# waleedbinkhalid74/cnn-gp

Measured on AMD Instinct MI355X. Metric: kernel entries/s (N×M pairs) + full-Kxx build+solve wall-clock, MNIST 28×28, higher is better.
Workload: dtype f64; 1 GPU; mnist_paper_convnet_gp Kxx 4096x4096, tiles 1024; n=4096, tile=1024, parallelism=tiles-dp1

## Files before the change

cnn-gp_amd/cnn_gp/_native.py:

```python
from __future__ import annotations

import ctypes
import os
import threading

_HERE = os.path.dirname(os.path.abspath(__file__))
LIB_PATH = os.environ.get("CNNGP_LIB",
                          os.path.join(os.path.dirname(_HERE), "lib", "libcnngp.so"))

CGP_ABI_VERSION = 12
CGP_FLAG_EXACT_RELU = 1
CGP_FLAG_GENERIC_CONV = 2
CGP_FLAG_NET_DUAL = 4
CGP_PRE_NONE, CGP_PRE_RELU, CGP_PRE_MOMENTS = 0, 1, 2
CGP_POST_NONE, CGP_POST_RELU = 0, 1
CGP_NET_CONV, CGP_NET_RELU, CGP_NET_MOMENTS, CGP_NET_LINEAR = 0, 1, 2, 3
CGP_NET_LOAD, CGP_NET_STORE = 4, 5
CGP_NET_CODE_HS_CLEAN = 0x100
CGP_NET_CODE_SUM = 0x200
CGP_NET_CODE_FROM_SUM = 0x400
CGP_NET_CODE_GEOMETRY = 0xff
CGP_VAR_MOMENTS, CGP_VAR_CONV, CGP_VAR_HALF, CGP_VAR_SUM = 0, 1, 2, 3
CGP_VAR_FORM_SCALED, CGP_VAR_FORM_RSQRT = 0, 1

_vp = ctypes.c_void_p
_i64 = ctypes.c_int64
_i32 = ctypes.c_int32
_f64 = ctypes.c_double


class ConvArgs(ctypes.Structure):
    _fields_ = [
        ("in_", _vp), ("in_y", _vp), ("out", _vp), ("addend", _vp),
        ("pre_xx", _vp), ("pre_yy", _vp), ("post_xx", _vp), ("post_yy", _vp),
        ("nmaps", _i64), ("n1", _i64), ("n2", _i64),
        ("h", _i32), ("w", _i32), ("ho", _i32), ("wo", _i32),
        ("taps", _i32), ("offset", _i32), ("stride", _i32), ("dilation", _i32),
        ("channels", _i32), ("pre", _i32), ("post", _i32), ("same", _i32), ("diag", _i32),
        ("maps_per_block", _i32), ("flags", _i32), ("reserved", _i32),
        ("weight", _f64), ("bias", _f64),
    ]


class ReluArgs(ctypes.Structure):
    _fields_ = [
        ("xy", _vp), ("out", _vp), ("addend", _vp), ("xx", _vp), ("yy", _vp),
        ("nmaps", _i64), ("n1", _i64), ("n2", _i64),
        ("hw", _i32), ("same", _i32), ("diag", _i32), ("flags", _i32),
    ]


class ReluNtkArgs(ctypes.Structure):
    _fields_ = [
        ("xy", _vp), ("theta", _vp), ("out_xy", _vp), ("out_theta", _vp),
        ("xx", _vp), ("yy", _vp),
        ("nmaps", _i64), ("n1", _i64), ("n2", _i64),
        ("hw", _i32), ("same", _i32), ("diag", _i32), ("flags", _i32),
    ]


class ErfArgs(ctypes.Structure):
    _fields_ = [
        ("xy", _vp), ("theta", _vp), ("out_xy", _vp), ("out_theta", _vp), ("addend", _vp),
        ("xx", _vp), ("yy", _vp),
        ("nmaps", _i64), ("n1", _i64), ("n2", _i64),
        ("hw", _i32), ("same", _i32), ("diag", _i32), ("flags", _i32),
    ]


class NetOp(ctypes.Structure):
    _fields_ = [
        ("kind", _i32), ("code", _i32), ("src", _i32), ("dst", _i32), ("add", _i32),
        ("ws_in", _i32), ("ws_out", _i32), ("relu", _i32), ("h", _i32), ("w", _i32),
        ("div_m", ctypes.c_uint32), ("div_s", ctypes.c_uint32),
        ("dst2", _i32), ("zero_halo", _i32),
        ("weight", _f64), ("bias", _f64), ("var_x", _vp), ("var_y", _vp),
        ("var2_x", _vp), ("var2_y", _vp),
    ]


class VarOp(ctypes.Structure):
    _fields_ = [
        ("kind", _i32), ("dst", _i32), ("src", _i32 * 4),
        ("h", _i32), ("w", _i32), ("ho", _i32), ("wo", _i32),
        ("taps", _i32), ("offset", _i32), ("stride", _i32), ("dilation", _i32),
        ("store", _i64), ("qstore", _i64),
        ("weight", _f64), ("bias", _f64), ("coef", _f64 * 4),
    ]


class VarArgs(ctypes.Structure):
    _fields_ = [
        ("x", _vp), ("y", _vp), ("out", _vp), ("ops", _vp),
        ("n1", _i64), ("n2", _i64), ("store_total", _i64),
        ("nops", _i32), ("channels", _i32), ("h", _i32), ("w", _i32),
        ("lds_elems", _i32), ("scratch", _i32),
    ]


class NetArgs(ctypes.Structure):
    _fields_ = [
        ("x", _vp), ("y", _vp), ("out", _vp), ("kdiag", _vp), ("ops", _vp),
        ("n1", _i64), ("n2", _i64), ("ldo", _i64),
        ("nops", _i32), ("channels", _i32), ("h", _i32), ("w", _i32),
        ("same", _i32), ("final_slot", _i32), ("hs", _i32), ("lds_elems", _i32),
        ("flags", _i32), ("pairs", _i32), ("unit_begin", _i64), ("unit_end", _i64),
        ("final_stage", _i32), ("program", _i32), ("part", _i32),
    ]


def make_fastdiv(d: int):
    s = 0
    while (1 << s) < d:
        s += 1
    m = (((1 << 32) * ((1 << s) - d)) // d + 1) & 0xFFFFFFFF
    return m, s


SIGNATURES = {
    "cgp_abi_version": (_i32, []),
    "cgp_net_xvar_scale": (ctypes.c_double, []),
    "cgp_net_var_form": (_i32, []),
    "cgp_last_error": (ctypes.c_char_p, []),
    "cgp_conv_args_size": (ctypes.c_size_t, []),
    "cgp_relu_args_size": (ctypes.c_size_t, []),
    "cgp_device_count": (_i32, []),
    "cgp_selftest": (_i32, []),
    "cgp_moments_xy_f64": (_i32, [_vp, _vp, _i64, _i64, _i32, _i32, _i32, _vp, _vp]),
    "cgp_moments_xy_f32": (_i32, [_vp, _vp, _i64, _i64, _i32, _i32, _i32, _vp, _vp]),
    "cgp_moments_var_f64": (_i32, [_vp, _vp, _i64, _i64, _i32, _i32, _vp, _vp, _vp]),
    "cgp_moments_var_f32": (_i32, [_vp, _vp, _i64, _i64, _i32, _i32, _vp, _vp, _vp]),
    "cgp_conv_f64": (_i32, [ctypes.POINTER(ConvArgs), _vp]),
    "cgp_conv_f32": (_i32, [ctypes.POINTER(ConvArgs), _vp]),
    "cgp_relu_f64": (_i32, [ctypes.POINTER(ReluArgs), _vp]),
    "cgp_relu_f32": (_i32, [ctypes.POINTER(ReluArgs), _vp]),
    "cgp_relu_ntk_args_size": (ctypes.c_size_t, []),
    "cgp_relu_ntk_f64": (_i32, [ctypes.POINTER(ReluNtkArgs), _vp]),
    "cgp_relu_ntk_f32": (_i32, [ctypes.POINTER(ReluNtkArgs), _vp]),
    "cgp_erf_args_size": (ctypes.c_size_t, []),
    "cgp_erf_f64": (_i32, [ctypes.POINTER(ErfArgs), _vp]),
    "cgp_erf_f32": (_i32, [ctypes.POINTER(ErfArgs), _vp]),
    "cgp_var_erf_f64": (_i32, [_vp, _vp, _i64, _i64, _i32, _i32, _vp, _vp, _vp]),
    "cgp_var_erf_f32": (_i32, [_vp, _vp, _i64, _i64, _i32, _i32, _vp, _vp, _vp]),
    "cgp_var_relu_f64": (_i32, [_vp, _vp, _i64, _i64, _i32, _i32, _vp, _vp, _vp]),
    "cgp_var_relu_f32": (_i32, [_vp, _vp, _i64, _i64, _i32, _i32, _vp, _vp, _vp]),
    "cgp_axpby_f64": (_i32, [_f64, _vp, _f64, _vp, _vp, _i64, _vp]),
    "cgp_axpby_f32": (_i32, [_f64, _vp, _f64, _vp, _vp, _i64, _vp]),
    "cgp_scale_batch_f64": (_i32, [_i32, _vp, _vp, _vp, _f64, _vp]),
    "cgp_rsqrt_batch_f64": (_i32, [_i32, _vp, _vp, _vp, _vp]),
    "cgp_cast_f32_f64": (_i32, [_vp, _vp, _i64, _vp]),
    "cgp_transpose_f64": (_i32, [_vp, _i64, _i64, _vp, _vp]),
    "cgp_chol_solve_f64": (_i32, [_vp, _i64, _i64, _vp, _i64, _i64, _f64,
                                  ctypes.POINTER(_i64), _vp]),
    "cgp_chol_last_phases": (_i32, [_vp, ctypes.POINTER(_f64)]),
    "cgp_chol_solve_f64_timed": (_i32, [_vp, _i64, _i64, _vp, _i64, _i64, _f64,
                                        ctypes.POINTER(_i64), ctypes.POINTER(_f64), _vp]),
    "cgp_gemm_f64": (_i32, [_vp, _vp, _vp, _i64, _i64, _i64, _vp]),
    "cgp_sym_mirror_f64": (_i32, [_vp, _i64, _i64, _vp, _vp]),
    "cgp_sym_residual_f64": (_i32, [_vp, _i64, _i64, _vp, _vp, _vp, _i64, _i64, _vp, _vp]),
    "cgp_argmax_rows_f64": (_i32, [_vp, _i64, _i64, _vp, _vp]),
    "cgp_pred_var_f64": (_i32, [_vp, _i64, _i64, _vp, _i64, _i64, _vp, _vp, _vp]),
    "cgp_net_geometry": (_i32, [_i32] * 7),
    "cgp_net_hs_elems": (_i32, [_i32]),
    "cgp_net_supertile": (_i32, []),
    "cgp_net_units": (_i32, [_i32]),
    "cgp_net_resolution": (_i32, [_i32, _i32]),
    "cgp_net_op_size": (ctypes.c_size_t, []),
    "cgp_net_args_size": (ctypes.c_size_t, []),
    "cgp_net_occupancy": (_i32, [_i32, _i32, _i32, _i32]),
    "cgp_net_program": (_i32, [_vp, _i32, _i32, _i32, _i32, _i32]),
    "cgp_net_validate": (_i32, [_vp, _i32, _i32]),
    "cgp_net_static_lds": (_i32, []),
    "cgp_net_f64": (_i32, [ctypes.POINTER(NetArgs), _vp]),
    "cgp_net_f32": (_i32, [ctypes.POINTER(NetArgs), _vp]),
    "cgp_var_op_size": (ctypes.c_size_t, []),
    "cgp_var_args_size": (ctypes.c_size_t, []),
    "cgp_var_chain_f64": (_i32, [ctypes.POINTER(VarArgs), _vp]),
    "cgp_var_chain_f32": (_i32, [ctypes.POINTER(VarArgs), _vp]),
}

_lib = None
_lib_err = None
_lock = threading.Lock()


def load():
    global _lib, _lib_err
    with _lock:
        if _lib is not None:
            return _lib
        if _lib_err is not None:
            raise RuntimeError(_lib_err)
        if not os.path.exists(LIB_PATH):
            _lib_err = (f"libcnngp.so not found at {LIB_PATH}: build it with "
                        "`python -c 'import __graft_entry__ as g; g.build()'` or "
                        "`make -C cnn-gp_amd/csrc` (no CPU fallback exists)")
            raise RuntimeError(_lib_err)
        try:
            lib = ctypes.CDLL(LIB_PATH)
        except OSError as e:
            _lib_err = f"failed to load {LIB_PATH}: {e}"
            raise RuntimeError(_lib_err) from e
        for name, (res, args) in SIGNATURES.items():
            fn = getattr(lib, name)
            fn.restype = res
            fn.argtypes = args
        if lib.cgp_abi_version() != CGP_ABI_VERSION:
            _lib_err = "libcnngp.so ABI version mismatch (rebuild it)"
            raise RuntimeError(_lib_err)
        if lib.cgp_conv_args_size() != ctypes.sizeof(ConvArgs) or \
                lib.cgp_relu_args_size() != ctypes.sizeof(ReluArgs) or \
                lib.cgp_relu_ntk_args_size() != ctypes.sizeof(ReluNtkArgs) or \
                lib.cgp_erf_args_size() != ctypes.sizeof(ErfArgs) or \
                lib.cgp_net_op_size() != ctypes.sizeof(NetOp) or \
                lib.cgp_net_args_size() != ctypes.sizeof(NetArgs) or \
                lib.cgp_var_op_size() != ctypes.sizeof(VarOp) or \
                lib.cgp_var_args_size() != ctypes.sizeof(VarArgs):
            _lib_err = "libcnngp.so argument struct layout differs from _native.py"
            raise RuntimeError(_lib_err)
        _lib = lib
        return lib


def check(rc: int, what: str):
    if rc != 0:
        msg = load().cgp_last_error().decode(errors="replace")
        raise RuntimeError(f"{what} failed (code {rc}): {msg}")


def call(name: str, *args):
    lib = load()
    check(getattr(lib, name)(*args), name)


def ptr(t):
    return None if t is None else ctypes.c_void_p(t.data_ptr())
```

cnn-gp_amd/csrc/cgp_common.h:

```cpp
#pragma once

#include <hip/hip_runtime.h>

#include <string>

#include "cnngp.h"
#include "relu_poly.h"

namespace cgp {

int fail(int code, const char* fmt, ...);
int check_launch(const char* what);
int device_cus();
inline hipStream_t as_stream(void* s) { return reinterpret_cast<hipStream_t>(s); }
inline hipError_t stream_device(hipStream_t s, int* dev) {
    if (s == nullptr) return hipGetDevice(dev);
    hipDevice_t d = 0;
    const hipError_t e = hipStreamGetDevice(s, &d);
    if (e == hipSuccess) *dev = (int)d;
    return e;
}

#define CGP_HIP(call)                                                                  \
    do {                                                                               \
        hipError_t e_ = (call);                                                        \
        if (e_ != hipSuccess)                                                          \
            return fail(CGP_EHIP, "%s: %s (%s:%d)", #call, hipGetErrorString(e_),      \
                        __FILE__, __LINE__);                                           \
    } while (0)


struct FastDiv {
    unsigned m, s, d;
};
__host__ __device__ inline FastDiv make_fastdiv(unsigned d) {
    FastDiv f;
    f.d = d;
    f.s = 0;
    while ((1ull << f.s) < d) ++f.s;
    f.m = (unsigned)(((1ull << 32) * ((1ull << f.s) - d)) / d + 1);
    return f;
}
__host__ __device__ __forceinline__ unsigned umulhi32(unsigned a, unsigned b) {
#ifdef __HIP_DEVICE_COMPILE__
    return __umulhi(a, b);
#else
    return (unsigned)(((unsigned long long)a * b) >> 32);
#endif
}
__host__ __device__ __forceinline__ unsigned fdiv(unsigned n, const FastDiv& f) {
    return (umulhi32(n, f.m) + n) >> f.s;
}

template <typename T> struct K;
template <> struct K<double> {
    static constexpr double pi = 3.141592653589793;
    static constexpr double two_pi = 6.283185307179586;
    static constexpr double tiny = 1.1754943508222875e-38;
    static constexpr double xfloor = 1e-300;
};
template <> struct K<float> {
    static constexpr float pi = 3.14159265358979f;
    static constexpr float two_pi = 6.28318530717959f;
    static constexpr float tiny = 1.17549435e-38f;
    static constexpr float xfloor = 1e-30f;
};

__device__ __forceinline__ double sqrt_t(double x) { return __builtin_sqrt(x); }
__device__ __forceinline__ float sqrt_t(float x) { return __builtin_sqrtf(x); }
__device__ __forceinline__ double acos_t(double x) { return acos(x); }
__device__ __forceinline__ float acos_t(float x) { return acosf(x); }

template <typename T>
__device__ __forceinline__ T relu_exact_inl(T c, T v1, T v2) {
    const T t = v1 * v2 + K<T>::tiny;
    T cs = c * (T(1) / sqrt_t(t));
    cs = cs < T(-1) ? T(-1) : (cs > T(1) ? T(1) : cs);
    T d = t - c * c;
    d = d < T(0) ? T(0) : d;
    const T s = sqrt_t(d);
    const T th = acos_t(cs);
    return (s + (K<T>::pi - th) * c) / K<T>::two_pi;
}
template <typename T>
__device__ __noinline__ T relu_exact(T c, T v1, T v2) {
    return relu_exact_inl(c, v1, v2);
}

__device__ __forceinline__ double rsqrt_fast(double t) {
    const double y = __builtin_amdgcn_rsq(t);
    const double e = __builtin_fma(-t * y, y, 1.0);
    return __builtin_fma(0.5 * y, e, y);
}
__device__ __forceinline__ float rsqrt_fast(float t) { return __builtin_amdgcn_rsqf(t); }
__device__ __forceinline__ double sqrt_fast(double x) {
    const double r = __builtin_amdgcn_rsq(x);
    const double s0 = x * r;
    return __builtin_fma(0.5 * r, __builtin_fma(-s0, s0, x), s0);
}
__device__ __forceinline__ float sqrt_fast(float x) { return x * __builtin_amdgcn_rsqf(x); }
__device__ __forceinline__ double relu_poly(double x) {
    double r = kReluPolyD[kReluPolyDegD];
#pragma unroll
    for (int k = kReluPolyDegD - 1; k >= 0; --k) r = __builtin_fma(r, x, kReluPolyD[k]);
    return r;
}
__device__ __forceinline__ float relu_poly(float x) {
    float r = kReluPolyF[kReluPolyDegF];
#pragma unroll
    for (int k = kReluPolyDegF - 1; k >= 0; --k) r = __builtin_fmaf(r, x, kReluPolyF[k]);
    return r;
}
__device__ __forceinline__ double fmin_t(double a, double b) { return __builtin_fmin(a, b); }
__device__ __forceinline__ float fmin_t(float a, float b) { return __builtin_fminf(a, b); }
__device__ __forceinline__ double fmax_t(double a, double b) { return __builtin_fmax(a, b); }
__device__ __forceinline__ float fmax_t(float a, float b) { return __builtin_fmaxf(a, b); }
__device__ __forceinline__ double fabs_t(double a) { return __builtin_fabs(a); }
__device__ __forceinline__ float fabs_t(float a) { return __builtin_fabsf(a); }
__device__ __forceinline__ double fma_t(double a, double b, double c) {
    return __builtin_fma(a, b, c);
}
__device__ __forceinline__ float fma_t(float a, float b, float c) {
    return __builtin_fmaf(a, b, c);
}

constexpr double kXVarScale = 0.0625;
#ifndef CGP_RELU_ONE_ROOT
#define CGP_RELU_ONE_ROOT 1
#endif
constexpr int kNetVarForm = CGP_RELU_ONE_ROOT ? CGP_VAR_FORM_RSQRT : CGP_VAR_FORM_SCALED;
constexpr double kPolyQ = CGP_RELU_ONE_ROOT ? 0.5 : 0.125;
__device__ __forceinline__ double var_rsqrt8(double v) { return 1.0 / __builtin_sqrt(v * 0.125); }
constexpr double kYMax = 0x1p66;
constexpr double poly_q(int k) {
    double v = kReluPolyD[k] * kPolyQ;
    for (int n = 0; n < k; ++n) v *= 0.25;
    return v;
}
struct PolyCoef {
    double c[kReluPolyDegD + 1];
};
constexpr PolyCoef poly_coef(bool quartered) {
    PolyCoef t{};
    for (int k = 0; k <= kReluPolyDegD; ++k) t.c[k] = quartered ? poly_q(k) : kReluPolyD[k];
    return t;
}
static __constant__ PolyCoef kReluPolyTabD = poly_coef(false);
static __constant__ PolyCoef kReluPolyTabDq = poly_coef(true);

template <int D>
struct AdaptCoef {
    double c[D + 1];
};
template <int D>
constexpr AdaptCoef<D> adapt_coef(const double (&p)[D + 1]) {
    AdaptCoef<D> t{};
    for (int k = 0; k <= D; ++k) {
        double v = p[k] * kPolyQ;
        for (int n = 0; n < k; ++n) v *= 0.25;
        t.c[k] = v;
    }
    return t;
}
static __constant__ AdaptCoef<kReluAdaptDeg0> kReluAdaptTab0 = adapt_coef<kReluAdaptDeg0>(kReluAdaptP0);
static __constant__ AdaptCoef<kReluAdaptDeg1> kReluAdaptTab1 = adapt_coef<kReluAdaptDeg1>(kReluAdaptP1);
static __constant__ AdaptCoef<kReluAdaptDeg2> kReluAdaptTab2 = adapt_coef<kReluAdaptDeg2>(kReluAdaptP2);

typedef const __attribute__((address_space(4))) double* ConstD;
struct PolyTab {
    ConstD d, dq;
    ConstD a0, a1, a2;
};
__device__ __forceinline__ PolyTab poly_table() {
    ConstD p = (ConstD)kReluPolyTabD.c;
    ConstD q = (ConstD)kReluPolyTabDq.c;
    asm volatile("" : "+s"(p), "+s"(q));
    ConstD a0 = (ConstD)kReluAdaptTab0.c;
    ConstD a1 = (ConstD)kReluAdaptTab1.c;
    ConstD a2 = (ConstD)kReluAdaptTab2.c;
    asm volatile("" : "+s"(a0), "+s"(a1), "+s"(a2));
    return PolyTab{p, q, a0, a1, a2};
}
__device__ __forceinline__ double fma_sc(double r, double u, double c) {
    double o;
    asm("v_fma_f64 %0, %1, %2, %3" : "=v"(o) : "v"(r), "v"(u), "s"(c));
    return o;
}
__device__ __forceinline__ double relu_poly(double x, const PolyTab& t) {
    double r = fma_sc(t.d[kReluPolyDegD], x, t.d[kReluPolyDegD - 1]);
#pragma unroll
    for (int k = kReluPolyDegD - 2; k >= 0; --k) r = fma_sc(r, x, t.d[k]);
    return r;
}
__device__ __forceinline__ float relu_poly(float x, const PolyTab&) { return relu_poly(x); }

template <typename T>
__device__ __forceinline__ T relu_fast(T c, T v1, T v2, const PolyTab& tab) {
    const T t = fma_t(v1, v2, K<T>::tiny);
    const T y = rsqrt_fast(t);
    const T st = t * y;
    const T a = fmin_t(fabs_t(c * y), T(1));
    const T x = fma_t(T(-0.5), a, T(0.5));
    const T sx = sqrt_fast(fmax_t(x, K<T>::xfloor));
    const T p = relu_poly(x, tab);
    const T hpos = (c + fabs_t(c)) * T(0.25);
    return fma_t((st * x) * sx, p, hpos);
}

constexpr double kRhoMax = 1.0 - 0x1p-52;
template <int R>
__device__ __forceinline__ void relu_fast_n(double (&c)[R], const double (&v1)[R],
                                            const double (&v2)[R], const PolyTab& tab) {
    double y[R], st[R], a[R], sx[R], u[R], p[R];
#pragma unroll
    for (int r = 0; r < R; ++r) {
        const double t = __builtin_fma(v1[r], v2[r], K<double>::tiny);
        y[r] = rsqrt_fast(t);
        st[r] = t * y[r];
    }
#pragma unroll
    for (int r = 0; r < R; ++r) {
        a[r] = __builtin_fmin(__builtin_fabs(c[r] * y[r]), kRhoMax);
        u[r] = __builtin_fma(-0.5, a[r], 0.5);
        sx[r] = (st[r] * u[r]) * sqrt_fast(u[r]);
    }
#pragma unroll
    for (int r = 0; r < R; ++r) p[r] = fma_sc(tab.d[kReluPolyDegD], u[r], tab.d[kReluPolyDegD - 1]);
#pragma unroll
    for (int k = kReluPolyDegD - 2; k >= 0; --k) {
        const double ck = tab.d[k];
#pragma unroll
        for (int r = 0; r < R; ++r) p[r] = fma_sc(p[r], u[r], ck);
    }
#pragma unroll
    for (int r = 0; r < R; ++r)
        c[r] = __builtin_fma(sx[r], p[r], (c[r] + __builtin_fabs(c[r])) * 0.25);
}
template <int R, int D>
__device__ __forceinline__ void horner_q(double (&p)[R], const double (&u)[R], ConstD t) {
#pragma unroll
    for (int r = 0; r < R; ++r) p[r] = fma_sc(t[D], u[r], t[D - 1]);
#pragma unroll
    for (int k = D - 2; k >= 0; --k) {
        const double ck = t[k];
#pragma unroll
        for (int r = 0; r < R; ++r) p[r] = fma_sc(p[r], u[r], ck);
    }
}
#ifndef CGP_RELU_VOTE_HI
#define CGP_RELU_VOTE_HI 1
#endif
__device__ __forceinline__ unsigned vote_hi(double v) {
    return (unsigned)(__builtin_bit_cast(unsigned long long, v) >> 32);
}
template <int R>
__device__ __forceinline__ unsigned vote_hi_max(const double (&u)[R]) {
    unsigned m = vote_hi(u[0]);
#pragma unroll
    for (int r = 1; r < R; ++r) m = m > vote_hi(u[r]) ? m : vote_hi(u[r]);
    return m;
}
template <int R, bool QIN, int AD = 0>
__device__ __forceinline__ void relu_q_n(double (&c)[R], const double (&v1q)[R],
                                         const double (&v2)[R], const PolyTab& tab,
                                         unsigned long long seg = ~0ull) {
    double sx[R], u[R], p[R];
#if CGP_RELU_ONE_ROOT
    double Y[R];
#pragma unroll
    for (int r = 0; r < R; ++r) {
        if constexpr (!QIN) c[r] *= 0.25;
        Y[r] = __builtin_fmin(v1q[r] * v2[r], kYMax);
    }
#pragma unroll
    for (int r = 0; r < R; ++r) {
        u[r] = __builtin_fmax(__builtin_fma(-__builtin_fabs(c[r]), Y[r], 2.0), 2.0 - 2.0 * kRhoMax);
        const double z = (u[r] * Y[r]) * Y[r];
        const double h = __builtin_amdgcn_rsq(z);
        const double m = z * h;
        const double R2 = h * __builtin_fma(-m, h, 3.0);
        sx[r] = (u[r] * u[r]) * R2;
    }
#else
    double y[R], st[R];
#pragma unroll
    for (int r = 0; r < R; ++r) {
        if constexpr (!QIN) c[r] *= 0.25;
        const double T = __builtin_fma(v1q[r], v2[r], kXVarScale * K<double>::tiny);
        const double r0 = __builtin_amdgcn_rsq(T);
        const double m = T * r0;
        const double k = __builtin_fma(-m, r0, 3.0);
        y[r] = r0 * k;
        st[r] = m * k;
    }
#pragma unroll
    for (int r = 0; r < R; ++r) {
        u[r] = __builtin_fmax(__builtin_fma(-__builtin_fabs(c[r]), y[r], 2.0), 2.0 - 2.0 * kRhoMax);
        const double h = __builtin_amdgcn_rsq(u[r]);
        const double m = u[r] * h;
        const double sq4 = m * __builtin_fma(-m, h, 3.0);
        sx[r] = (st[r] * u[r]) * sq4;
    }
#endif
    if constexpr (AD == 2) {
        const unsigned long long ex = __builtin_amdgcn_read_exec() & seg;
        auto all_seg = [&](bool pred) { return (__ballot(pred) & seg) == ex; };
#if CGP_RELU_VOTE_HI
        const unsigned hm = vote_hi_max<R>(u);
        if (all_seg(hm < vote_hi(4.0 * kReluAdaptX0))) {
            horner_q<R, kReluAdaptDeg0>(p, u, tab.a0);
        } else if (all_seg(hm < vote_hi(4.0 * kReluAdaptX1))) {
            horner_q<R, kReluAdaptDeg1>(p, u, tab.a1);
        } else if (all_seg(hm < vote_hi(4.0 * kReluAdaptX2))) {
#else
        double um = u[0];
#pragma unroll
        for (int r = 1; r < R; ++r) um = __builtin_fmax(um, u[r]);
        if (all_seg(um <= 4.0 * kReluAdaptX0)) {
            horner_q<R, kReluAdaptDeg0>(p, u, tab.a0);
        } else if (all_seg(um <= 4.0 * kReluAdaptX1)) {
            horner_q<R, kReluAdaptDeg1>(p, u, tab.a1);
        } else if (all_seg(um <= 4.0 * kReluAdaptX2)) {
#endif
            horner_q<R, kReluAdaptDeg2>(p, u, tab.a2);
        } else {
            horner_q<R, kReluPolyDegD>(p, u, tab.dq);
        }
    } else if constexpr (AD == 1) {
#if CGP_RELU_VOTE_HI
        const unsigned hm = vote_hi_max<R>(u);
        if (__all(hm < vote_hi(4.0 * kReluAdaptX0))) {
            horner_q<R, kReluAdaptDeg0>(p, u, tab.a0);
        } else if (__all(hm < vote_hi(4.0 * kReluAdaptX1))) {
            horner_q<R, kReluAdaptDeg1>(p, u, tab.a1);
        } else if (__all(hm < vote_hi(4.0 * kReluAdaptX2))) {
#else
        double um = u[0];
#pragma unroll
        for (int r = 1; r < R; ++r) um = __builtin_fmax(um, u[r]);
        if (__all(um <= 4.0 * kReluAdaptX0)) {
            horner_q<R, kReluAdaptDeg0>(p, u, tab.a0);
        } else if (__all(um <= 4.0 * kReluAdaptX1)) {
            horner_q<R, kReluAdaptDeg1>(p, u, tab.a1);
        } else if (__all(um <= 4.0 * kReluAdaptX2)) {
#endif
            horner_q<R, kReluAdaptDeg2>(p, u, tab.a2);
        } else {
            horner_q<R, kReluPolyDegD>(p, u, tab.dq);
        }
    } else {
        horner_q<R, kReluPolyDegD>(p, u, tab.dq);
    }
#pragma unroll
    for (int r = 0; r < R; ++r) c[r] = __builtin_fma(sx[r], p[r], c[r] + __builtin_fabs(c[r]));
}
typedef float cgp_f2 __attribute__((ext_vector_type(2)));
__device__ __forceinline__ cgp_f2 relu_fast2(cgp_f2 c, cgp_f2 v1, cgp_f2 v2) {
    const cgp_f2 t = __builtin_elementwise_fma(v1, v2, cgp_f2(K<float>::tiny));
    const cgp_f2 y = {__builtin_amdgcn_rsqf(t.x), __builtin_amdgcn_rsqf(t.y)};
    const cgp_f2 st = t * y;
    const cgp_f2 cy = c * y;
    const cgp_f2 a = {__builtin_fminf(__builtin_fabsf(cy.x), 1.0f),
                      __builtin_fminf(__builtin_fabsf(cy.y), 1.0f)};
    const cgp_f2 x = __builtin_elementwise_fma(cgp_f2(-0.5f), a, cgp_f2(0.5f));
    const cgp_f2 xm = {__builtin_fmaxf(x.x, K<float>::xfloor), __builtin_fmaxf(x.y, K<float>::xfloor)};
    const cgp_f2 h = {__builtin_amdgcn_rsqf(xm.x), __builtin_amdgcn_rsqf(xm.y)};
    const cgp_f2 sx = xm * h;
    cgp_f2 p = cgp_f2(kReluPolyF[kReluPolyDegF]);
#pragma unroll
    for (int k = kReluPolyDegF - 1; k >= 0; --k)
        p = __builtin_elementwise_fma(p, x, cgp_f2(kReluPolyF[k]));
    const cgp_f2 ac = {__builtin_fabsf(c.x), __builtin_fabsf(c.y)};
    const cgp_f2 hpos = (c + ac) * cgp_f2(0.25f);
    return __builtin_elementwise_fma((st * x) * sx, p, hpos);
}
__device__ __forceinline__ void relu_prep2(cgp_f2 c, cgp_f2 v1, cgp_f2 v2, cgp_f2& x, cgp_f2& m,
                                           cgp_f2& hpos) {
    const cgp_f2 t = __builtin_elementwise_fma(v1, v2, cgp_f2(K<float>::tiny));
    const cgp_f2 y = {__builtin_amdgcn_rsqf(t.x), __builtin_amdgcn_rsqf(t.y)};
    const cgp_f2 st = t * y;
    const cgp_f2 cy = c * y;
    const cgp_f2 a = {__builtin_fminf(__builtin_fabsf(cy.x), 1.0f),
                      __builtin_fminf(__builtin_fabsf(cy.y), 1.0f)};
    x = __builtin_elementwise_fma(cgp_f2(-0.5f), a, cgp_f2(0.5f));
    const cgp_f2 xm = {__builtin_fmaxf(x.x, K<float>::xfloor), __builtin_fmaxf(x.y, K<float>::xfloor)};
    const cgp_f2 h = {__builtin_amdgcn_rsqf(xm.x), __builtin_amdgcn_rsqf(xm.y)};
    m = (st * x) * (xm * h);
    const cgp_f2 ac = {__builtin_fabsf(c.x), __builtin_fabsf(c.y)};
    hpos = (c + ac) * cgp_f2(0.25f);
}
__device__ __forceinline__ void relu_prep1(float c, float v1, float v2, float& x, float& m,
                                           float& hpos) {
    const float t = __builtin_fmaf(v1, v2, K<float>::tiny);
    const float y = __builtin_amdgcn_rsqf(t);
    const float st = t * y;
    const float a = __builtin_fminf(__builtin_fabsf(c * y), 1.0f);
    x = __builtin_fmaf(-0.5f, a, 0.5f);
    const float xm = __builtin_fmaxf(x, K<float>::xfloor);
    m = (st * x) * (xm * __builtin_amdgcn_rsqf(xm));
    hpos = (c + __builtin_fabsf(c)) * 0.25f;
}
template <int R, int D>
__device__ __forceinline__ void relu_poly_f(const float (&P)[D + 1], float (&c)[R],
                                            const cgp_f2 (&x2)[R / 2 + 1],
                                            const cgp_f2 (&m2)[R / 2 + 1],
                                            const cgp_f2 (&h2)[R / 2 + 1], float xs, float ms,
                                            float hs) {
#pragma unroll
    for (int q = 0; q < R / 2; ++q) {
        cgp_f2 p = cgp_f2(P[D]);
#pragma unroll
        for (int k = D - 1; k >= 0; --k) p = __builtin_elementwise_fma(p, x2[q], cgp_f2(P[k]));
        const cgp_f2 o = __builtin_elementwise_fma(m2[q], p, h2[q]);
        c[2 * q] = o.x;
        c[2 * q + 1] = o.y;
    }
    if constexpr (R % 2) {
        float p = P[D];
#pragma unroll
        for (int k = D - 1; k >= 0; --k) p = __builtin_fmaf(p, xs, P[k]);
        c[R - 1] = __builtin_fmaf(ms, p, hs);
    }
}
template <int R>
__device__ __forceinline__ void relu_fast_n(float (&c)[R], const float (&v1)[R],
                                            const float (&v2)[R], const PolyTab&) {
    cgp_f2 x2[R / 2 + 1], m2[R / 2 + 1], h2[R / 2 + 1];
    float xs = 0.0f, ms = 0.0f, hs = 0.0f;
#pragma unroll
    for (int q = 0; q < R / 2; ++q)
        relu_prep2(cgp_f2{c[2 * q], c[2 * q + 1]}, cgp_f2{v1[2 * q], v1[2 * q + 1]},
                   cgp_f2{v2[2 * q], v2[2 * q + 1]}, x2[q], m2[q], h2[q]);
    if constexpr (R % 2) relu_prep1(c[R - 1], v1[R - 1], v2[R - 1], xs, ms, hs);
    relu_poly_f<R, kReluPolyDegF>(kReluPolyF, c, x2, m2, h2, xs, ms, hs);
}

template <typename T>
__device__ __forceinline__ T relu_fast(T c, T v1, T v2) {
    const T t = v1 * v2 + K<T>::tiny;
    const T y = rsqrt_fast(t);
    const T st = t * y;
    const T a = fmin_t(fabs_t(c * y), T(1));
    const T x = fma_t(T(-0.5), a, T(0.5));
    const T sx = sqrt_fast(fmax_t(x, K<T>::xfloor));
    const T p = relu_poly(x);
    const T pos = fmax_t(c, T(0));
    return fma_t((st * x) * sx, p, T(0.5) * pos) + (c - c);
}

template <typename T>
__device__ __forceinline__ T relu_pair(T c, const T* __restrict__ xx, const T* __restrict__ yy,
                                       unsigned i, unsigned j, int hw, int px, int same,
                                       int diag, int exact) {
    const T v1 = xx[(size_t)i * hw + px];
    if (same && (diag || i == j)) return v1 / T(2);
    const T v2 = yy[(size_t)j * hw + px];
    return exact ? relu_exact(c, v1, v2) : relu_fast(c, v1, v2);
}

__device__ __forceinline__ double atan_t(double x) { return atan(x); }
__device__ __forceinline__ float atan_t(float x) { return atanf(x); }

template <typename T> struct KErf {
    static constexpr T two_over_pi = T(0.63661977236758134308);
    static constexpr T four_over_pi = T(1.27323954473516268615);
};

template <typename T>
__device__ __forceinline__ T erf_var(T v, T& kdot) {
    const T s = sqrt_t(T(1) + T(4) * v);
    kdot = KErf<T>::four_over_pi / s;
    return KErf<T>::two_over_pi * atan_t((T(2) * v) / s);
}
template <typename T>
__device__ __forceinline__ T erf_var(T v) {
    T kdot;
    return erf_var(v, kdot);
}

template <typename T>
__device__ __forceinline__ T erf_pair(T c, const T* __restrict__ xx, const T* __restrict__ yy,
                                      unsigned i, unsigned j, int hw, int px, int same,
                                      int diag, T& kdot) {
    const T v1 = xx[(size_t)i * hw + px];
    if (same && (diag || i == j)) return erf_var(v1, kdot);
    const T v2 = yy[(size_t)j * hw + px];
    T d = T(1) + T(2) * (v1 + v2) + T(4) * (v1 * v2 - c * c);
    d = d < T(1) ? T(1) : d;
    const T s = sqrt_t(d);
    kdot = KErf<T>::four_over_pi / s;
    return KErf<T>::two_over_pi * atan_t((T(2) * c) / s);
}

__device__ __forceinline__ void pair_of(unsigned m, const FastDiv& n2, int diag, unsigned& i,
                                        unsigned& j) {
    if (diag) {
        i = j = m;
    } else {
        i = fdiv(m, n2);
        j = m - i * n2.d;
    }
}

__device__ __forceinline__ void lds_barrier() {
    asm volatile("s_waitcnt lgkmcnt(0)" ::: "memory");
    __builtin_amdgcn_s_barrier();
    asm volatile("" ::: "memory");
}

}
```

cnn-gp_amd/csrc/netfuse.hip:

```cpp

#include "cgp_common.h"


#include <map>
#include <mutex>
#include <utility>
#include <algorithm>
#include <climits>

using namespace cgp;

namespace {

constexpr int kNT = 128;
constexpr int kSplit = 2;
template <int NP>
constexpr int kNTof = NP == 2 ? kSplit * kNT : kNT;
template <int NP>
constexpr int kUnitsOf = NP == 2 ? kSplit : NP;
constexpr int kSTL = 3;
constexpr int kST = 1 << kSTL;
constexpr int kEw = 4;

constexpr int pick_r(int lines, int len, int taps, int s, int epi, int nt) {
    int best = 1;
    long long best_cost = LLONG_MAX;
    for (int r = 1; r <= 8 && r <= len; ++r) {
        if (len % r) continue;
        const int items = lines * (len / r);
        const int rounds = (items + nt - 1) / nt;
        const long long cost = (long long)rounds * (epi * r + (r - 1) * s + taps);
        if (cost < best_cost || (cost == best_cost && r > best)) {
            best = r;
            best_cost = cost;
        }
    }
    return best;
}

template <int H_, int W_, int HO_, int WO_, int TAPS_, int S_, int OFF_, int NP_ = 1>
struct NG {
    static constexpr int H = H_, W = W_, HO = HO_, WO = WO_, TAPS = TAPS_, S = S_, OFF = OFF_;
    static constexpr int NP = NP_;
    static constexpr int NT = kNT;
    static_assert(NP_ != 2, "two-pair workgroups run their ops as one-pair halves");
    static constexpr int HW = H * W, HOWO = HO * WO;
    static constexpr bool POINT = TAPS == 1 && OFF == 0;
    static constexpr bool REDUCE = HO == 1 && WO == 1 && OFF == 0 && TAPS == H && TAPS == W;
    static constexpr int HSR = (HO - 1) * S + TAPS;
    static constexpr int Q0 = OFF < 0 ? -OFF : 0;
    static constexpr int Q1 = HSR < H - OFF ? HSR : H - OFF;
    static constexpr int NVR = Q1 - Q0;
    static constexpr int R2 = pick_r(NVR * NP, WO, TAPS, S, 2, NT);
    static constexpr int R3 = pick_r(WO * NP, HO, TAPS, S, 8, NT);
    static constexpr int WIN2 = (R2 - 1) * S + TAPS, WIN3 = (R3 - 1) * S + TAPS;
    static constexpr int NG2 = WO / R2, NH = NVR * NG2, KH = (NP * NH + NT - 1) / NT;
    static constexpr int NG3 = HO / R3, NV = NG3 * WO, KV = (NP * NV + NT - 1) / NT;
    static constexpr int NZ = (HSR - NVR) * WO;
    static constexpr bool DIRECT = !POINT && !REDUCE && TAPS <= 3;
    static constexpr int HS_ELEMS = (POINT || REDUCE || DIRECT) ? 2 : HSR * WO;
};

#define CGP_NET_GEOMETRIES(X)          \
    X(28, 28, 28, 28, 7, 1, -3)        \
    X(28, 28, 28, 28, 4, 1, -1)        \
    X(28, 28, 28, 28, 3, 1, -1)        \
    X(28, 28, 28, 28, 1, 1, 0)         \
    X(28, 28, 14, 14, 3, 2, -1)        \
    X(28, 28, 14, 14, 1, 2, 0)         \
    X(28, 28, 1, 1, 28, 1, 0)          \
    X(14, 14, 14, 14, 3, 1, -1)        \
    X(14, 14, 7, 7, 3, 2, -1)          \
    X(14, 14, 7, 7, 1, 2, 0)           \
    X(7, 7, 7, 7, 3, 1, -1)            \
    X(7, 7, 1, 1, 7, 1, 0)             \
    X(1, 1, 1, 1, 1, 1, 0)             \
    X(32, 32, 32, 32, 3, 1, -1)        \
    X(32, 32, 32, 32, 1, 1, 0)         \
    X(32, 32, 16, 16, 3, 2, -1)        \
    X(32, 32, 16, 16, 1, 2, 0)         \
    X(16, 16, 16, 16, 3, 1, -1)        \
    X(16, 16, 8, 8, 3, 2, -1)          \
    X(16, 16, 8, 8, 1, 2, 0)           \
    X(8, 8, 8, 8, 3, 1, -1)            \
    X(8, 8, 1, 1, 8, 1, 0)             \
    X(14, 14, 1, 1, 14, 1, 0)          \
    X(16, 16, 1, 1, 16, 1, 0)          \
    X(32, 32, 1, 1, 32, 1, 0)

struct GeoRow {
    int h, w, ho, wo, taps, s, off, hs_elems;
};
#define CGP_NET_ROW(h, w, ho, wo, k, s, o) {h, w, ho, wo, k, s, o, NG<h, w, ho, wo, k, s, o>::HS_ELEMS},
constexpr GeoRow kGeoTable[] = {CGP_NET_GEOMETRIES(CGP_NET_ROW)};
#undef CGP_NET_ROW
constexpr int kNumGeo = sizeof(kGeoTable) / sizeof(kGeoTable[0]);

template <typename T, int TAPS, int O0, int G, int N, int R>
__device__ __forceinline__ void win_group(const T (&w)[N], T (&out)[R]) {
    T core = w[O0 + G - 1];
#pragma unroll
    for (int t = O0 + G; t < O0 + TAPS; ++t) core += w[t];
    if constexpr (G == 1) {
        out[O0] = core;
    } else {
        T suf[G], right[G];
        suf[G - 1] = core;
#pragma unroll
        for (int o = G - 2; o >= 0; --o) suf[o] = w[O0 + o] + suf[o + 1];
        right[1] = w[O0 + TAPS];
#pragma unroll
        for (int o = 2; o < G; ++o) right[o] = right[o - 1] + w[O0 + TAPS + o - 1];
        out[O0] = suf[0];
#pragma unroll
        for (int o = 1; o < G; ++o) out[O0 + o] = suf[o] + right[o];
    }
}

template <typename T, int TAPS, int O0, int N, int R>
__device__ __forceinline__ void win_groups(const T (&w)[N], T (&out)[R]) {
    if constexpr (O0 < R) {
        constexpr int G = (R - O0) < TAPS ? (R - O0) : TAPS;
        win_group<T, TAPS, O0, G, N, R>(w, out);
        win_groups<T, TAPS, O0 + TAPS, N, R>(w, out);
    }
}

template <typename T, int TAPS, int S, int R>
__device__ __forceinline__ void win_sums(const T (&w)[(R - 1) * S + TAPS], T (&out)[R]) {
    if constexpr (S == 1 && TAPS >= 4 && R > 1) {
        win_groups<T, TAPS, 0, (R - 1) * S + TAPS, R>(w, out);
    } else {
#pragma unroll
        for (int o = 0; o < R; ++o) {
            T acc = w[o * S];
#pragma unroll
            for (int t = 1; t < TAPS; ++t) acc += w[o * S + t];
            out[o] = acc;
        }
    }
}

__device__ __forceinline__ int opaque_tid() {
    static_assert(kNT == 128, "opaque_tid masks to 128-thread halves");
    int t;
    asm volatile("v_and_b32 %0, 0x7f, %1" : "=v"(t) : "v"((int)threadIdx.x));
    return t;
}

__device__ __forceinline__ int udiv(int a, int d) { return (int)((unsigned)a / (unsigned)d); }

typedef const cgp_net_op* OpsC;
__device__ __forceinline__ OpsC ops_c(const cgp_net_op* p) { return (OpsC)p; }
__device__ __forceinline__ cgp_net_op load_op(OpsC r) {
    cgp_net_op o;
    o.kind = r->kind;
    o.code = r->code;
    o.src = r->src;
    o.dst = r->dst;
    o.add = r->add;
    o.ws_in = r->ws_in;
    o.ws_out = r->ws_out;
    o.relu = r->relu;
    o.h = r->h;
    o.w = r->w;
    o.div_m = r->div_m;
    o.div_s = r->div_s;
    o.dst2 = r->dst2;
    o.zero_halo = r->zero_halo;
    o.weight = r->weight;
    o.bias = r->bias;
    o.var_x = r->var_x;
    o.var_y = r->var_y;
    o.var2_x = r->var2_x;
    o.var2_y = r->var2_y;
    return o;
}

template <typename T>
using GP = const __attribute__((address_space(1))) T*;
template <typename T>
__device__ __forceinline__ GP<T> gptr(const void* p) {
    return (GP<T>)(const T*)p;
}

template <typename T>
__device__ __forceinline__ T wave_sum(T v) {
#pragma unroll
    for (int m = 32; m >= 1; m >>= 1) v += __shfl_xor(v, m, 64);
    return v;
}

template <typename T>
struct NetP {
    const T* __restrict__ x;
    const T* __restrict__ y;
    T* __restrict__ out;
    const T* __restrict__ kdiag;
    const cgp_net_op* __restrict__ ops;
    unsigned long long* work;
    long long ldo, units, ubeg, uend;
    unsigned n1, n2, nbi, nbj;
    int nops, channels, hw_in, same, final_slot, hs, lds_elems, exact, final_stage, part;
};

constexpr int kMaxNP = 16;
constexpr long long kStaticLds = 1536;
struct Pairs {
    unsigned i, j;
    const unsigned* tab;
    long long u0;
    void* red;
};
template <int NP>
__device__ __forceinline__ void pair_q(const Pairs& pr, int q, unsigned& iq, unsigned& jq) {
    if constexpr (NP == 1) {
        iq = pr.i;
        jq = pr.j;
    } else {
        iq = pr.tab[q];
        jq = pr.tab[kMaxNP + q];
    }
}

template <bool EXACT, typename T>
__device__ __forceinline__ T relu_of(T c, T v1, T v2, const PolyTab& tab) {
    if constexpr (EXACT)
        return relu_exact_inl(c, v1, v2);
    else
        return relu_fast(c, v1, v2, tab);
}
template <typename T, bool EX>
constexpr bool kQuarter = !EX && sizeof(T) == 8;

template <bool EXACT, bool QIN, typename T, int R, int AD = 0>
__device__ __forceinline__ void relu_n(T (&v)[R], const T (&u1)[R], const T (&u2)[R],
                                       const PolyTab& tab, unsigned long long seg = ~0ull) {
    if constexpr (EXACT) {
#pragma unroll
        for (int k = 0; k < R; ++k) v[k] = relu_exact_inl(v[k], u1[k], u2[k]);
    } else if constexpr (sizeof(T) == 8) {
        relu_q_n<R, QIN, AD>(v, u1, u2, tab, seg);
    } else {
        relu_fast_n<R>(v, u1, u2, tab);
    }
}

#define CGP_NET_RESOLUTIONS(X) X(28, 28) X(14, 14) X(7, 7) X(32, 32) X(16, 16) X(8, 8) X(1, 1)

struct ResRow {
    int h, w;
};
#define CGP_NET_RES_ROW(h, w) {h, w},
constexpr ResRow kResTable[] = {CGP_NET_RESOLUTIONS(CGP_NET_RES_ROW)};
#undef CGP_NET_RES_ROW
constexpr int kNumRes = sizeof(kResTable) / sizeof(kResTable[0]);
constexpr int res_index(int h, int w) {
    for (int n = 0; n < kNumRes; ++n)
        if (kResTable[n].h == h && kResTable[n].w == w) return n;
    return -1;
}

template <typename T, bool EX, bool DU, int R, int AD = 0>
__device__ __forceinline__ void net_out(T* __restrict__ lds, const cgp_net_op& op, T (&v)[R],
                                        const int (&at)[R], const bool (&ok)[R],
                                        const T (&u1)[R], const T (&u2)[R],
                                        const PolyTab& tab, unsigned long long seg = ~0ull) {
    if (op.relu) relu_n<EX, kQuarter<T, EX>, T, R, AD>(v, u1, u2, tab, seg);
    if (op.add >= 0) {
#pragma unroll
        for (int k = 0; k < R; ++k)
            if (ok[k]) v[k] += lds[op.add + at[k]];
    }
#pragma unroll
    for (int k = 0; k < R; ++k)
        if (ok[k]) lds[op.dst + at[k]] = v[k];
    if (DU && op.dst2 >= 0) {
        relu_n<EX, false, T, R, AD>(v, u1, u2, tab, seg);
#pragma unroll
        for (int k = 0; k < R; ++k)
            if (ok[k]) lds[op.dst2 + at[k]] = v[k];
    }
}

__device__ __forceinline__ GP<char> ubase(const void* p) {
    const unsigned long long v = (unsigned long long)p;
    const unsigned lo = __builtin_amdgcn_readfirstlane((unsigned)v);
    const unsigned hi = __builtin_amdgcn_readfirstlane((unsigned)(v >> 32));
    return (GP<char>)(const char*)(((unsigned long long)hi << 32) | lo);
}

template <typename T>
struct VarSrc {
    GP<char> x, y;
    unsigned xo, yo;
    bool on;
    __device__ __forceinline__ T ldx(unsigned px, int k = 0) const {
        return *(GP<T>)(x + (size_t)(xo + px * (unsigned)sizeof(T)) + k * (int)sizeof(T));
    }
    __device__ __forceinline__ T ldy(unsigned px, int k = 0) const {
        return *(GP<T>)(y + (size_t)(yo + px * (unsigned)sizeof(T)) + k * (int)sizeof(T));
    }
};
template <typename T, bool UNI>
__device__ __forceinline__ VarSrc<T> var_maps(const void* vx, const void* vy, bool on,
                                              unsigned i, unsigned j, int hw) {
    VarSrc<T> r;
    r.on = on;
    r.x = ubase(vx);
    r.y = ubase(vy);
    if constexpr (UNI) {
        r.x += (size_t)i * (size_t)hw * sizeof(T);
        r.y += (size_t)j * (size_t)hw * sizeof(T);
        r.xo = r.yo = 0;
    } else {
        r.xo = i * (unsigned)hw * (unsigned)sizeof(T);
        r.yo = j * (unsigned)hw * (unsigned)sizeof(T);
    }
    return r;
}
template <typename T, bool UNI>
__device__ __forceinline__ VarSrc<T> var_src(const cgp_net_op& op, unsigned i, unsigned j,
                                             int hw) {
    const bool two = op.dst2 >= 0;
    return var_maps<T, UNI>(two ? op.var2_x : op.var_x, two ? op.var2_y : op.var_y,
                            op.relu != 0 || two, i, j, hw);
}

template <int NP>
constexpr int kAdaptOf = NP == 1 ? 1 : 2;
constexpr int kPrio = 2;
constexpr int kPrioMaxHW = 28 * 28;
template <int NP, int HW>
constexpr bool kPrioOn = HW <= kPrioMaxHW;
template <int NP, int HW>
__device__ __forceinline__ void prio_mem() {
    if constexpr (kPrioOn<NP, HW>) __builtin_amdgcn_s_setprio(kPrio);
}
template <int NP, int HW>
__device__ __forceinline__ void prio_alu() {
    if constexpr (kPrioOn<NP, HW>) __builtin_amdgcn_s_setprio(0);
}
template <int PER, int NPR>
struct VoteCuts {
    int n = 0;
    int at[64] = {};
    constexpr VoteCuts() {
        for (int off = 1; off < PER && n < 64; ++off) {
            bool cut = false;
            for (int k = 1; 64 * k < NPR * PER; ++k) cut = cut || (64 * k) % PER == off;
            if (cut) at[n++] = off;
        }
    }
};
template <int PER, int NPR>
__device__ __forceinline__ unsigned long long vote_lanes(int it) {
    constexpr VoteCuts<PER, NPR> cuts{};
    const int wb = it & ~63, q = udiv(it, PER), l = it - q * PER;
    int lo = 0, hi = PER;
#pragma unroll
    for (int k = 0; k < cuts.n; ++k) {
        if (cuts.at[k] <= l) lo = cuts.at[k];
        if (cuts.at[k] > l && cuts.at[k] < hi) hi = cuts.at[k];
    }
    int a = q * PER + lo - wb, b = q * PER + hi - wb;
    a = a < 0 ? 0 : a;
    b = b > 64 ? 64 : b;
    const unsigned long long top = b >= 64 ? ~0ull : ((1ull << b) - 1ull);
    return top & ~((1ull << a) - 1ull);
}
#ifndef CGP_NET_RES_UNDEF
#define CGP_NET_RES_UNDEF 1
#endif
template <typename T, bool EX, bool DU, class G, bool PRE = false>
__device__ __forceinline__ void net_conv(T* __restrict__ lds, const cgp_net_op& op,
                                         const NetP<T>& p, const Pairs& pr) {
    constexpr int NP = G::NP;
    const int tid = opaque_tid();
    const PolyTab tab = poly_table();
    const T qs = !PRE && kQuarter<T, EX> && op.relu ? T(0.25) : T(1);
    const T w = T(op.weight) * qs, b = T(op.bias) * qs;
    const int arena = NP == 1 ? 0 : p.lds_elems;
    prio_mem<NP, G::HW>();
    const VarSrc<T> vs0 = var_src<T, NP == 1>(op, pr.i, pr.j, G::HOWO);
    auto vs_of = [&](int q) {
        if constexpr (NP == 1) {
            return vs0;
        } else {
            unsigned iq, jq;
            pair_q<NP>(pr, q, iq, jq);
            return var_src<T, false>(op, iq, jq, G::HOWO);
        }
    };
    const T* __restrict__ src = lds + op.src;
    const int wsi = op.ws_in, wso = op.ws_out;

    if constexpr (G::REDUCE && NP == 1) {
        prio_alu<NP, G::HW>();
        const bool from_sum = (op.code & CGP_NET_CODE_FROM_SUM) != 0;
        T* part = from_sum ? static_cast<T*>(pr.red)
                           : lds + p.part;
        if (!from_sum) {
            T acc = T(0);
#pragma unroll
            for (int k = 0; k < (G::HW + G::NT - 1) / G::NT; ++k) {
                const int px = tid + k * G::NT;
                if (G::HW % G::NT == 0 || px < G::HW) {
                    const int r = udiv(px, G::W), c = px - r * G::W;
                    acc += src[r * wsi + c];
                }
            }
            acc = wave_sum(acc);
            if ((tid & 63) == 0) part[tid >> 6] = acc;
            lds_barrier();
        }
        if (tid == 0) {
            T tot = part[0];
#pragma unroll
            for (int k = 1; k < G::NT / 64; ++k) tot += part[k];
            T v[1] = {fma_t(w, tot, b)};
            const int at[1] = {0};
            const bool ok[1] = {true};
            T u1[1] = {T(1)}, u2[1] = {T(1)};
            if (vs0.on) {
                u1[0] = vs0.ldx(0);
                u2[0] = vs0.ldy(0);
            }
            net_out<T, EX, DU, 1>(lds, op, v, at, ok, u1, u2, tab);
        }
    } else if constexpr (G::REDUCE) {
        prio_alu<NP, G::HW>();
        constexpr int TPP = G::NT / NP;
        static_assert(TPP <= 64 && G::NT % NP == 0, "reduce groups must not straddle waves");
        const int q = udiv(tid, TPP), lane = tid - q * TPP;
        const T* srcq = src + q * arena;
        T acc = T(0);
#pragma unroll
        for (int k = 0; k < (G::HW + TPP - 1) / TPP; ++k) {
            const int px = lane + k * TPP;
            if (G::HW % TPP == 0 || px < G::HW) {
                const int r = udiv(px, G::W), c = px - r * G::W;
                acc += srcq[r * wsi + c];
            }
        }
#pragma unroll
        for (int m = TPP / 2; m >= 1; m >>= 1) acc += __shfl_xor(acc, m, 64);
        if (lane == 0) {
            const VarSrc<T> vs = vs_of(q);
            T v[1] = {fma_t(w, acc, b)};
            const int at[1] = {q * arena};
            const bool ok[1] = {true};
            T u1[1] = {T(1)}, u2[1] = {T(1)};
            if (vs.on) {
                u1[0] = vs.ldx(0);
                u2[0] = vs.ldy(0);
            }
            net_out<T, EX, DU, 1>(lds, op, v, at, ok, u1, u2, tab);
        }
    } else if constexpr (G::POINT) {
        prio_alu<NP, G::HW>();
        constexpr int N = NP * G::HOWO;
        constexpr int KP = (N + G::NT - 1) / G::NT;
        T u1[KP], u2[KP], v[KP];
        int at[KP];
        bool ok[KP];
#pragma unroll
        for (int k = 0; k < KP; ++k) {
            const int e = tid + k * G::NT;
            ok[k] = N % G::NT == 0 || e < N;
            const int ec = ok[k] ? e : 0;
            const int q = NP == 1 ? 0 : udiv(ec, G::HOWO), pc = ec - q * G::HOWO;
            const int r = udiv(pc, G::WO), c = pc - r * G::WO;
            const VarSrc<T> vs = vs_of(q);
            at[k] = q * arena + r * wso + c;
            u1[k] = (vs.on && ok[k]) ? vs.ldx((unsigned)pc) : T(1);
            u2[k] = (vs.on && ok[k]) ? vs.ldy((unsigned)pc) : T(1);
            v[k] = fma_t(w, src[q * arena + (r * G::S) * wsi + c * G::S], b);
        }
        net_out<T, EX, DU, KP, NP == 1 ? 1 : 0>(lds, op, v, at, ok, u1, u2, tab);
    } else if constexpr (G::DIRECT) {
        constexpr int NVT = NP * G::NV;
        T u1[G::KV][G::R3], u2[G::KV][G::R3];
#pragma unroll
        for (int kv = 0; kv < G::KV; ++kv) {
            const int it = tid + kv * G::NT;
            const int itc = (NVT % G::NT == 0 || it < NVT) ? it : 0;
            const int q = NP == 1 ? 0 : udiv(itc, G::NV), l = itc - q * G::NV;
            const int g3 = udiv(l, G::WO), c = l - g3 * G::WO;
            const VarSrc<T> vs = vs_of(q);
#pragma unroll
            for (int k = 0; k < G::R3; ++k) {
                const unsigned px0 = (unsigned)(g3 * G::R3 * G::WO + c);
                u1[kv][k] = vs.on ? vs.ldx(px0, k * G::WO) : T(1);
                u2[kv][k] = vs.on ? vs.ldy(px0, k * G::WO) : T(1);
            }
        }
        const int s_lo = op.src - wsi, s_hi = op.src + G::H * wsi;
        auto hits = [&](int d) {
            return d >= 0 && d - wso < s_hi && d + G::HO * wso > s_lo;
        };
        const bool hazard = hits(op.dst) || (DU && hits(op.dst2));
        T res[G::KV][G::R3];
#if CGP_NET_RES_UNDEF
#pragma unroll
        for (int kv = 0; kv < G::KV; ++kv)
#pragma unroll
            for (int k = 0; k < G::R3; ++k) asm volatile("" : "=v"(res[kv][k]));
#endif
#pragma unroll
        for (int kv = 0; kv < G::KV; ++kv) {
            const int it = tid + kv * G::NT;
            if (NVT % G::NT == 0 || it < NVT) {
                const int q = NP == 1 ? 0 : udiv(it, G::NV), l = it - q * G::NV;
                const int g3 = udiv(l, G::WO), c = l - g3 * G::WO;
                const T* base = src + q * arena + c * G::S + G::OFF;
                const int r0 = g3 * G::R3 * G::S + G::OFF;
                T rs[G::WIN3];
#pragma unroll
                for (int t = 0; t < G::WIN3; ++t) {
                    const bool lo = G::OFF + t < 0, hi = (G::NG3 - 1) * G::R3 * G::S + G::OFF + t >= G::H;
                    const int r = r0 + t;
                    const bool in = (!lo || r >= 0) && (!hi || r < G::H);
                    const T* row = base + (in ? r : 0) * wsi;
                    T a = row[0];
#pragma unroll
                    for (int dx = 1; dx < G::TAPS; ++dx) a += row[dx];
                    rs[t] = in ? a : T(0);
                }
                T o[G::R3];
                win_sums<T, G::TAPS, G::S, G::R3>(rs, o);
#pragma unroll
                for (int k = 0; k < G::R3; ++k) res[kv][k] = fma_t(w, o[k], b);
#pragma unroll
                for (int k = 0; k < G::R3; ++k)
                    asm volatile("" : "+v"(u1[kv][k]), "+v"(u2[kv][k]));
            }
        }
        prio_alu<NP, G::HW>();
        if (hazard) lds_barrier();
#pragma unroll
        for (int kv = 0; kv < G::KV; ++kv) {
            const int it = tid + kv * G::NT;
            if (NVT % G::NT == 0 || it < NVT) {
                const int q = NP == 1 ? 0 : udiv(it, G::NV), l = it - q * G::NV;
                const int g3 = udiv(l, G::WO), c = l - g3 * G::WO;
                int at[G::R3];
                bool ok[G::R3];
#pragma unroll
                for (int k = 0; k < G::R3; ++k) {
                    at[k] = q * arena + (g3 * G::R3 + k) * wso + c;
                    ok[k] = true;
                }
                net_out<T, EX, DU, G::R3, kAdaptOf<NP>>(lds, op, res[kv], at, ok, u1[kv],
                                                        u2[kv], tab,
                                                        NP == 1 ? ~0ull : vote_lanes<G::NV, NP>(it));
            }
        }
    } else {
        T* __restrict__ hs = lds + p.hs;
        constexpr int NHT = NP * G::NH, NVT = NP * G::NV, NZT = NP * G::NZ;
        T u1[G::KV][G::R3], u2[G::KV][G::R3];
        if (vs0.on) {
#pragma unroll
            for (int kv = 0; kv < G::KV; ++kv) {
                const int it = tid + kv * G::NT;
                const int itc = (NVT % G::NT == 0 || it < NVT) ? it : 0;
                const int q = NP == 1 ? 0 : udiv(itc, G::NV), l = itc - q * G::NV;
                const int g3 = udiv(l, G::WO), c = l - g3 * G::WO;
                const VarSrc<T> vs = vs_of(q);
#pragma unroll
                for (int k = 0; k < G::R3; ++k) {
                    const unsigned px0 = (unsigned)(g3 * G::R3 * G::WO + c);
                    u1[kv][k] = vs.ldx(px0, k * G::WO);
                    u2[kv][k] = vs.ldy(px0, k * G::WO);
                }
            }
        } else {
#pragma unroll
            for (int kv = 0; kv < G::KV; ++kv)
#pragma unroll
                for (int k = 0; k < G::R3; ++k) u1[kv][k] = u2[kv][k] = T(1);
        }
#pragma unroll
        for (int kh = 0; kh < G::KH; ++kh) {
            const int it = tid + kh * G::NT;
            if (NHT % G::NT == 0 || it < NHT) {
                const int q = NP == 1 ? 0 : udiv(it, G::NH), l = it - q * G::NH;
                const int qi = udiv(l, G::NG2), g2 = l - qi * G::NG2;
                const T* row = lds + (op.src + q * arena + (G::Q0 + qi + G::OFF) * wsi +
                                      g2 * G::R2 * G::S + G::OFF);
                T win[G::WIN2];
#pragma unroll
                for (int t = 0; t < G::WIN2; ++t) win[t] = row[t];
                T o[G::R2];
                win_sums<T, G::TAPS, G::S, G::R2>(win, o);
                T* h = hs + q * arena + (G::Q0 + qi) * G::WO + g2 * G::R2;
#pragma unroll
                for (int t = 0; t < G::R2; ++t) h[t] = o[t];
            }
        }
        if constexpr (G::NZ > 0) {
            if (!(op.code & CGP_NET_CODE_HS_CLEAN)) {
#pragma unroll
                for (int z0 = 0; z0 < NZT; z0 += G::NT) {
                    const int z = z0 + tid;
                    if (NZT % G::NT == 0 || z < NZT) {
                        const int q = NP == 1 ? 0 : udiv(z, G::NZ), zl = z - q * G::NZ;
                        hs[q * arena + (zl < G::Q0 * G::WO ? zl : zl + G::NVR * G::WO)] = T(0);
                    }
                }
            }
        }
        lds_barrier();
        const bool to_sum = NP == 1 && (op.code & CGP_NET_CODE_SUM) != 0;
        T sacc = T(0);
#pragma unroll
        for (int kv = 0; kv < G::KV; ++kv) {
            const int it = tid + kv * G::NT;
            if (NVT % G::NT == 0 || it < NVT) {
                const int q = NP == 1 ? 0 : udiv(it, G::NV), l = it - q * G::NV;
                const int g3 = udiv(l, G::WO), c = l - g3 * G::WO;
                const T* col = lds + (p.hs + q * arena + g3 * G::R3 * G::S * G::WO + c);
                T win[G::WIN3];
#pragma unroll
                for (int t = 0; t < G::WIN3; ++t) win[t] = col[t * G::WO];
#pragma unroll
                for (int k = 0; k < G::R3; ++k) asm volatile("" : "+v"(u1[kv][k]), "+v"(u2[kv][k]));
                T o[G::R3], v[G::R3];
                win_sums<T, G::TAPS, G::S, G::R3>(win, o);
                prio_alu<NP, G::HW>();
                int at[G::R3];
                bool ok[G::R3];
#pragma unroll
                for (int k = 0; k < G::R3; ++k) {
                    v[k] = fma_t(w, o[k], b);
                    at[k] = q * arena + (g3 * G::R3 + k) * wso + c;
                    ok[k] = true;
                }
                if (to_sum) {
                    if (op.relu) relu_n<EX, kQuarter<T, EX>, T, G::R3, 1>(v, u1[kv], u2[kv], tab);
#pragma unroll
                    for (int k = 0; k < G::R3; ++k) sacc += v[k];
                } else {
                    net_out<T, EX, DU, G::R3, kAdaptOf<NP>>(lds, op, v, at, ok, u1[kv], u2[kv],
                                                            tab,
                                                            NP == 1 ? ~0ull
                                                                    : vote_lanes<G::NV, NP>(it));
                }
            }
        }
        if constexpr (NP == 1) {
            if (to_sum) {
                sacc = wave_sum(sacc);
                if ((tid & 63) == 0) static_cast<T*>(pr.red)[tid >> 6] = sacc;
            }
        }
    }
}

template <typename T, bool EX, bool DU, int KIND, int KE, int W_, int NP>
__device__ __forceinline__ void elem_pass(T* __restrict__ lds, const cgp_net_op& op,
                                          const NetP<T>& p, const Pairs& pr, int tid,
                                          int base, int hw, const PolyTab& tab) {
    static_assert(NP == 1 || W_ > 0, "multi-pair elementwise ops need a compile-time size");
    const int wd = W_ ? W_ : op.w, ws = op.ws_out;
    const int arena = NP == 1 ? 0 : p.lds_elems;
    const FastDiv fw{op.div_m, op.div_s, (unsigned)op.w};
    auto vs_of = [&](unsigned iq, unsigned jq) {
        return KIND == CGP_NET_RELU
                   ? var_maps<T, NP == 1>(op.var_x, op.var_y, true, iq, jq, hw)
                   : var_src<T, NP == 1>(op, iq, jq, hw);
    };
    const VarSrc<T> vs0 = vs_of(pr.i, pr.j);
    const GP<char> xi = ubase(p.x) + (size_t)pr.i * p.channels * hw * sizeof(T);
    const GP<char> yj = ubase(p.y) + (size_t)pr.j * p.channels * hw * sizeof(T);
    auto img = [](GP<char> b, unsigned e) {
        return *(GP<T>)(b + (size_t)(e * (unsigned)sizeof(T)));
    };
    const int n = NP * hw;
    const bool live = base + (tid & ~63) < n;
    T a[KE], u1[KE], u2[KE];
    int at[KE];
    bool ok[KE];
#pragma unroll
    for (int k = 0; k < KE; ++k) {
        const int e = base + k * kNT + tid;
        ok[k] = e < n;
        const int ec = ok[k] ? e : 0;
        const int q = NP == 1 ? 0 : ec / hw, pc = ec - q * hw;
        const int r = W_ ? udiv(pc, W_) : (int)fdiv((unsigned)pc, fw);
        at[k] = q * arena + r * ws + (pc - r * wd);
        VarSrc<T> vs = vs0;
        if constexpr (NP > 1) {
            unsigned iq, jq;
            pair_q<NP>(pr, q, iq, jq);
            vs = vs_of(iq, jq);
        }
        u1[k] = (vs.on && ok[k]) ? vs.ldx((unsigned)pc) : T(1);
        u2[k] = (vs.on && ok[k]) ? vs.ldy((unsigned)pc) : T(1);
        if constexpr (KIND == CGP_NET_RELU) {
            a[k] = lds[op.src + at[k]];
        } else if constexpr (KIND == CGP_NET_MOMENTS) {
            static_assert(NP == 1, "moments run one pair per workgroup (half)");
            T acc = img(xi, (unsigned)pc) * img(yj, (unsigned)pc);
            for (int ch = 1; ch < p.channels; ++ch) {
                const unsigned e = (unsigned)(ch * hw + pc);
                acc += img(xi, e) * img(yj, e);
            }
            a[k] = acc;
        } else {
            a[k] = T(op.weight) * lds[op.src + at[k]] + T(op.bias) * lds[op.add + at[k]];
        }
    }
    if constexpr (KIND == CGP_NET_MOMENTS) {
        if (p.channels != 1) {
#pragma unroll
            for (int k = 0; k < KE; ++k) a[k] = a[k] / T(p.channels);
        }
    }
    if constexpr (KIND == CGP_NET_RELU) {
        if (live) relu_n<EX, false, T, KE, NP == 1 ? 1 : 0>(a, u1, u2, tab);
        if (op.add >= 0) {
#pragma unroll
            for (int k = 0; k < KE; ++k)
                if (ok[k]) a[k] += lds[op.add + at[k]];
        }
    }
#pragma unroll
    for (int k = 0; k < KE; ++k)
        if (ok[k]) lds[op.dst + at[k]] = a[k];
    if constexpr (KIND == CGP_NET_LINEAR && DU) {
        if (op.dst2 >= 0) {
            if (live) relu_n<EX, false, T, KE, NP == 1 ? 1 : 0>(a, u1, u2, tab);
#pragma unroll
            for (int k = 0; k < KE; ++k)
                if (ok[k]) lds[op.dst2 + at[k]] = a[k];
        }
    }
}

template <typename T, bool EX, bool DU, int KIND, int H_, int W_, int NP, int PI>
__device__ __forceinline__ void elem_passes(T* __restrict__ lds, const cgp_net_op& op,
                                            const NetP<T>& p, const Pairs& pr, int tid,
                                            const PolyTab& tab) {
    constexpr int KF = (NP * H_ * W_ + kNT - 1) / kNT;
    if constexpr (PI * kEw < KF) {
        constexpr int KE = KF - PI * kEw < kEw ? KF - PI * kEw : kEw;
        elem_pass<T, EX, DU, KIND, KE, W_, NP>(lds, op, p, pr, tid, PI * kEw * kNT, H_ * W_,
                                               tab);
        elem_passes<T, EX, DU, KIND, H_, W_, NP, PI + 1>(lds, op, p, pr, tid, tab);
    }
}

template <typename T, bool EX, bool DU, int KIND, int H_, int W_, int NP>
__device__ __forceinline__ void net_elem(T* __restrict__ lds, const cgp_net_op& op,
                                         const NetP<T>& p, const Pairs& pr) {
    const int tid = opaque_tid();
    const PolyTab tab = poly_table();
    if constexpr (H_ == 0) {
        const int hw = op.h * op.w;
        for (int base = 0; base < hw; base += kEw * kNT)
            elem_pass<T, EX, DU, KIND, kEw, 0, 1>(lds, op, p, pr, tid, base, hw, tab);
    } else {
        elem_passes<T, EX, DU, KIND, H_, W_, NP, 0>(lds, op, p, pr, tid, tab);
    }
}

template <typename T, int KIND, int NP>
__device__ __forceinline__ void net_move(T* __restrict__ lds, const cgp_net_op& op,
                                         const NetP<T>& p, const Pairs& pr) {
    const int tid = opaque_tid();
    const int hw = op.h * op.w, n = NP * hw;
    const int arena = NP == 1 ? 0 : p.lds_elems;
    T* state = const_cast<T*>(static_cast<const T*>(op.var_x));
    for (int e = tid; e < n; e += kNT) {
        const int q = NP == 1 ? 0 : e / hw, l = e - q * hw;
        const int r = l / op.w, c = l - r * op.w;
        const size_t g = (size_t)(pr.u0 + q - p.ubeg) * (size_t)op.code + (size_t)op.add +
                         (size_t)l;
        if constexpr (KIND == CGP_NET_LOAD)
            lds[op.dst + q * arena + r * op.ws_out + c] = state[g];
        else
            state[g] = lds[op.src + q * arena + r * op.ws_in + c];
    }
}

#ifndef CGP_NET_MOVE_C
#define CGP_NET_MOVE_C 1
#endif
template <typename T, int KIND, int NP, int H_, int W_, int SLOT, int WS>
__device__ __forceinline__ void net_move_c(T* __restrict__ lds, const cgp_net_op& op,
                                           const NetP<T>& p, const Pairs& pr) {
    const int tid = opaque_tid();
    constexpr int HW = H_ * W_, N = NP * HW, KP = (N + kNT - 1) / kNT;
    const int arena = NP == 1 ? 0 : p.lds_elems;
    const unsigned long long u0 =
        ((unsigned long long)__builtin_amdgcn_readfirstlane((unsigned)((unsigned long long)pr.u0 >> 32)) << 32) |
        __builtin_amdgcn_readfirstlane((unsigned)pr.u0);
    const unsigned code = (unsigned)__builtin_amdgcn_readfirstlane(op.code);
    const GP<char> base = ubase(op.var_x) +
                          ((size_t)(u0 - (unsigned long long)p.ubeg) * code + (size_t)op.add) *
                              sizeof(T);
#pragma unroll
    for (int k = 0; k < KP; ++k) {
        const int e = k * kNT + tid;
        if (N % kNT == 0 || e < N) {
            const unsigned q = NP == 1 ? 0u : (unsigned)udiv(e, HW);
            const unsigned l = (unsigned)e - q * (unsigned)HW;
            const unsigned r = (unsigned)udiv((int)l, W_), c = l - r * (unsigned)W_;
            T* cell = lds + (SLOT + (int)q * arena + (int)(r * (unsigned)WS + c));
            typedef __attribute__((address_space(1))) T* GW;
            GW g = (GW)(base + (size_t)((q * code + l) * (unsigned)sizeof(T)));
            if constexpr (KIND == CGP_NET_LOAD)
                *cell = *g;
            else
                *g = *cell;
        }
    }
}

template <typename T, int NT>
__device__ __forceinline__ void zero_halos(T* lds, int origin, int code, int h, int w, int ws,
                                           int tid) {
    if (!code) return;
    const int hl = code >> 8, gap = code & 0xff;
    for (int e = tid; e < hl + h * gap; e += NT) {
        int cell;
        if (e < hl) {
            cell = origin - hl + e;
        } else {
            const int r = (e - hl) / gap;
            cell = origin + r * ws + w + (e - hl - r * gap);
        }
        lds[cell] = T(0);
    }
}

__device__ __forceinline__ void tri_decode(unsigned s, unsigned nb, unsigned& bi,
                                           unsigned& bj) {
    const double a = 2.0 * nb + 1.0;
    long long r = (long long)((a - sqrt(a * a - 8.0 * (double)s)) * 0.5);
    auto off = [nb](long long q) { return q * (long long)nb - q * (q - 1) / 2; };
    if (r < 0) r = 0;
    while (r > 0 && off(r) > (long long)s) --r;
    while (off(r + 1) <= (long long)s) ++r;
    bi = (unsigned)r;
    bj = (unsigned)(r + ((long long)s - off(r)));
}

template <typename T>
__device__ __forceinline__ bool unit_pair(const NetP<T>& p, long long u, unsigned& i,
                                          unsigned& j) {
    const unsigned s = (unsigned)(u >> (2 * kSTL)), q = (unsigned)u & (kST * kST - 1u);
    unsigned bi, bj;
    if (p.same) {
        tri_decode(s, p.nbi, bi, bj);
    } else {
        bi = s / p.nbj;
        bj = s - bi * p.nbj;
    }
    i = bi * kST + (q >> kSTL);
    j = bj * kST + (q & (kST - 1u));
    return u < p.units && i < p.n1 && j < p.n2;
}

constexpr int geo_index(int h, int w, int ho, int wo, int k, int s, int o) {
    for (int n = 0; n < kNumGeo; ++n) {
        const GeoRow& g = kGeoTable[n];
        if (g.h == h && g.w == w && g.ho == ho && g.wo == wo && g.taps == k && g.s == s &&
            g.off == o)
            return n;
    }
    return -1;
}

#define CGP_NET_FITS(h, w) (NP == 1 || (h) * (w) * NP <= 1024)

#define CGP_NET_CASE(h, w, ho, wo, k, s, o)                                          \
    case geo_index(h, w, ho, wo, k, s, o):                                           \
        if constexpr (CGP_NET_FITS(h, w))                                            \
            net_conv<T, EX, DU, NG<h, w, ho, wo, k, s, o, NP>>(lds, op, p, pr);      \
        break;

#define CGP_NET_RES_CASE(h, w)                                                        \
    case res_index(h, w):                                                             \
        if constexpr (CGP_NET_FITS(h, w)) net_elem<T, EX, DU, KIND, h, w, NP>(lds, op, p, pr); \
        break;

template <typename T, bool EX, bool DU, int KIND, int NP>
__device__ __forceinline__ void net_elem_dispatch(T* __restrict__ lds, const cgp_net_op& op,
                                                  const NetP<T>& p, const Pairs& pr) {
    if constexpr (KIND == CGP_NET_RELU || (KIND == CGP_NET_LINEAR && NP > 1)) {
        switch (op.code) {
            CGP_NET_RESOLUTIONS(CGP_NET_RES_CASE)
        default:
            if constexpr (NP == 1) net_elem<T, EX, DU, KIND, 0, 0, 1>(lds, op, p, pr);
            break;
        }
    } else if constexpr (NP == 1) {
        net_elem<T, EX, DU, KIND, 0, 0, 1>(lds, op, p, pr);
    }
}

template <typename T, bool EX, bool DU, int NP>
__device__ __forceinline__ void net_op(T* __restrict__ lds, const cgp_net_op& op,
                                       const NetP<T>& p, const Pairs& pr, int tid) {
    if (op.zero_halo) {
#pragma unroll
        for (int q = 0; q < NP; ++q) {
            const int qa = NP == 1 ? 0 : q * p.lds_elems;
            zero_halos<T, kNT>(lds + qa, op.dst, op.zero_halo & 0xffff, op.h, op.w,
                                     op.ws_out, tid);
            zero_halos<T, kNT>(lds + qa, op.dst2, (unsigned)op.zero_halo >> 16, op.h, op.w,
                       op.ws_out, tid);
        }
    }
    switch (op.kind) {
    case CGP_NET_CONV:
        switch (op.code & CGP_NET_CODE_GEOMETRY) {
            CGP_NET_GEOMETRIES(CGP_NET_CASE)
        default:
            break;
        }
        break;
    case CGP_NET_RELU:
        net_elem_dispatch<T, EX, DU, CGP_NET_RELU, NP>(lds, op, p, pr);
        break;
    case CGP_NET_MOMENTS:
        net_elem_dispatch<T, EX, DU, CGP_NET_MOMENTS, NP>(lds, op, p, pr);
        break;
    case CGP_NET_LINEAR:
        net_elem_dispatch<T, EX, DU, CGP_NET_LINEAR, NP>(lds, op, p, pr);
        break;
    case CGP_NET_LOAD:
        net_move<T, CGP_NET_LOAD, NP>(lds, op, p, pr);
        break;
    case CGP_NET_STORE:
        net_move<T, CGP_NET_STORE, NP>(lds, op, p, pr);
        break;
    default:
        break;
    }
}

#ifndef CGP_NET_PRESCALE
#define CGP_NET_PRESCALE 1
#endif
constexpr bool kNetPrescale = CGP_NET_PRESCALE != 0;
struct ProgOp {
    int kind, code, src, dst, add, ws_in, ws_out, relu, h, w, dst2, zero_halo;
};
struct ProgInfo {
    int first, nops, pairs, dual, lds_elems, sizes;
};
#include "net_programs.h"
constexpr int kNumProgs = sizeof(kProgs) / sizeof(kProgs[0]);

struct ProgRec {
    double weight, bias;
    const void* var_x;
    const void* var_y;
    const void* var2_x;
    const void* var2_y;
};
template <int PID>
constexpr int kRecsOf = PID >= 0 ? kProgs[PID < 0 ? 0 : PID].nops : 1;

template <int PID, int K>
__device__ __forceinline__ cgp_net_op prog_op(const ProgRec* recs) {
    constexpr ProgOp o = kProgOps[kProgs[PID].first + K];
    const ProgRec& rt = recs[K];
    cgp_net_op op;
    op.kind = o.kind;
    op.code = o.code;
    op.src = o.src;
    op.dst = o.dst;
    op.add = o.add;
    op.ws_in = o.ws_in;
    op.ws_out = o.ws_out;
    op.relu = o.relu;
    op.h = o.h;
    op.w = o.w;
    op.div_m = 0;
    op.div_s = 0;
    op.dst2 = o.dst2;
    op.zero_halo = o.zero_halo;
    op.weight = rt.weight;
    op.bias = rt.bias;
    op.var_x = rt.var_x;
    op.var_y = rt.var_y;
    op.var2_x = rt.var2_x;
    op.var2_y = rt.var2_y;
    return op;
}
template <int PID, int K, int NP>
struct ProgGeo {
    static constexpr ProgOp o = kProgOps[kProgs[PID].first + K];
    static constexpr GeoRow g = kGeoTable[o.code & CGP_NET_CODE_GEOMETRY];
    using G = NG<g.h, g.w, g.ho, g.wo, g.taps, g.s, g.off, NP>;
};
template <typename T, bool DU, int NP, int PID, int K>
__device__ __forceinline__ void prog_ops(T* __restrict__ lds, const NetP<T>& p, const Pairs& pr,
                                         int tid, const ProgRec* recs) {
    constexpr ProgInfo I = kProgs[PID];
    if constexpr (K < I.nops) {
        constexpr ProgOp o = kProgOps[I.first + K];
        const cgp_net_op op = prog_op<PID, K>(recs);
        if constexpr (o.zero_halo != 0) {
#pragma unroll
            for (int q = 0; q < NP; ++q) {
                const int qa = q * I.lds_elems;
                zero_halos<T, kNT>(lds + qa, o.dst, o.zero_halo & 0xffff, o.h, o.w,
                                         o.ws_out, tid);
                zero_halos<T, kNT>(lds + qa, o.dst2, (unsigned)o.zero_halo >> 16, o.h, o.w,
                                         o.ws_out,
                           tid);
            }
        }
        if constexpr (o.kind == CGP_NET_CONV) {
            net_conv<T, false, DU, typename ProgGeo<PID, K, NP>::G, kNetPrescale>(lds, op, p,
                                                                                 pr);
        } else if constexpr (o.kind == CGP_NET_RELU || o.kind == CGP_NET_LINEAR ||
                             o.kind == CGP_NET_MOMENTS) {
            net_elem<T, false, DU, o.kind, o.h, o.w, NP>(lds, op, p, pr);
        } else if constexpr (o.kind == CGP_NET_LOAD || o.kind == CGP_NET_STORE) {
            if constexpr (CGP_NET_MOVE_C)
                net_move_c<T, o.kind, NP, o.h, o.w, o.kind == CGP_NET_LOAD ? o.dst : o.src,
                           o.kind == CGP_NET_LOAD ? o.ws_out : o.ws_in>(lds, op, p, pr);
            else
                net_move<T, o.kind, NP>(lds, op, p, pr);
        }
        lds_barrier();
        prog_ops<T, DU, NP, PID, K + 1>(lds, p, pr, tid, recs);
    }
}

int prog_match(const cgp_net_op* ops, int nops, int pairs, int dual, int lds_elems,
               int itemsize) {
    for (int k = 0; k < kNumProgs; ++k) {
        const ProgInfo& I = kProgs[k];
        if (I.nops != nops || I.pairs != pairs || I.dual != dual || I.lds_elems != lds_elems ||
            !(I.sizes & itemsize))
            continue;
        bool eq = true;
        for (int n = 0; n < nops && eq; ++n) {
            const ProgOp& o = kProgOps[I.first + n];
            const cgp_net_op& r = ops[n];
            eq = o.kind == r.kind && o.code == r.code && o.src == r.src && o.dst == r.dst &&
                 o.add == r.add && o.ws_in == r.ws_in && o.ws_out == r.ws_out &&
                 o.relu == r.relu && o.h == r.h && o.w == r.w && o.dst2 == r.dst2 &&
                 o.zero_halo == r.zero_halo;
        }
        if (eq) return k + 1;
    }
    return 0;
}

template <typename T, bool EX, bool DU, int WPE, int NP, int PID = -1>
__global__ __launch_bounds__(kNTof<NP>) __attribute__((amdgpu_waves_per_eu(WPE))) void net_kernel(const NetP<T> p) {
    extern __shared__ __align__(16) unsigned char smem_raw[];
    __shared__ unsigned pair_tab[2 * kMaxNP];
    __shared__ T red_part[kUnitsOf<NP> * (kNT / 64)];
    T* lds = reinterpret_cast<T*>(smem_raw);
    const int tid = threadIdx.x;
    constexpr int UN = kUnitsOf<NP>;
    for (int e = tid; e < UN * p.lds_elems; e += kNTof<NP>) lds[e] = T(0);
    if (tid < UN * (kNT / 64)) red_part[tid] = T(0);
    __shared__ ProgRec prog_recs[kRecsOf<PID>];
    __shared__ long long next_u[2];
    static_assert(sizeof(pair_tab) + sizeof(red_part) + sizeof(prog_recs) + sizeof(next_u) <=
                      kStaticLds,
                  "static LDS beyond the reserve the host checks count (kStaticLds)");
    if constexpr (PID >= 0) {
        for (int k = tid; k < kRecsOf<PID>; k += kNTof<NP>) {
            const cgp_net_op& r = p.ops[k];
            const ProgOp& o = kProgOps[kProgs[PID < 0 ? 0 : PID].first + k];
            const double qs =
                kNetPrescale && kQuarter<T, false> && o.kind == CGP_NET_CONV && o.relu ? 0.25 : 1.0;
            prog_recs[k] = ProgRec{r.weight * qs, r.bias * qs, r.var_x, r.var_y, r.var2_x,
                                   r.var2_y};
        }
    }
    lds_barrier();
    const unsigned xcd = blockIdx.x % 8;
    const long long span = p.uend - p.ubeg;
    const long long per = ((span + 7) / 8 + UN - 1) / UN * UN;
    const long long beg = p.ubeg + (long long)xcd * per;
    const long long end = beg + per < p.uend ? beg + per : p.uend;
    int adv = 0;
    unsigned long long* ctr = p.work + xcd;
    unsigned long long grab = 0;
    if (tid == 0) grab = atomicAdd(ctr, 1ull);
    auto advance = [&]() {
        if (tid == 0) next_u[adv] = beg + (long long)grab * UN;
        lds_barrier();
        const long long v = next_u[adv];
        adv ^= 1;
        return v;
    };
    for (long long u = advance(); u < end; u = advance()) {
        if (tid == 0) grab = atomicAdd(ctr, 1ull);
        Pairs pr;
        pr.tab = pair_tab;
        pr.u0 = u;
        pr.red = red_part;
        if constexpr (NP == 2) {
            const int q = __builtin_amdgcn_readfirstlane(tid >> 7);
            unsigned iq = 0, jq = 0;
            bool vq = false, wq = false, any = false;
#pragma unroll
            for (int s = 0; s < UN; ++s) {
                unsigned is = 0, js = 0;
                const bool vs = u + s < end && unit_pair(p, u + s, is, js);
                const bool ws = vs && !(p.same && js <= is);
                any |= ws;
                if (s == q) {
                    iq = is;
                    jq = js;
                    vq = vs;
                    wq = ws;
                }
            }
            if (!any) {
                if (p.final_stage && p.same && (tid & (kNT - 1)) == 0 && vq && jq == iq)
                    p.out[(long long)iq * p.ldo + iq] = p.kdiag[iq];
                continue;
            }
            Pairs ph;
            ph.tab = pair_tab;
            ph.u0 = u + q;
            ph.red = red_part + q * (kNT / 64);
            ph.i = __builtin_amdgcn_readfirstlane(vq ? iq : 0u);
            ph.j = __builtin_amdgcn_readfirstlane(vq ? jq : 0u);
            T* lh = lds + q * p.lds_elems;
            const int ht = tid & (kNT - 1);
            if constexpr (PID < 0) {
                for (int k = 0; k < p.nops; ++k) {
                    const cgp_net_op op = load_op(ops_c(p.ops) + k);
                    net_op<T, EX, DU, 1>(lh, op, p, ph, ht);
                    lds_barrier();
                }
            } else {
                prog_ops<T, DU, 1, PID, 0>(lh, p, ph, ht, prog_recs);
            }
            if (p.final_stage && ht == 0 && vq) {
                if (wq) {
                    const T v = lh[p.final_slot];
                    p.out[(long long)ph.i * p.ldo + ph.j] = v;
                    if (p.same) p.out[(long long)ph.j * p.ldo + ph.i] = v;
                } else if (ph.j == ph.i) {
                    p.out[(long long)ph.i * p.ldo + ph.i] = p.kdiag[ph.i];
                }
            }
        } else {
            if constexpr (NP == 1) {
                if (!unit_pair(p, u, pr.i, pr.j)) continue;
                pr.i = __builtin_amdgcn_readfirstlane(pr.i);
                pr.j = __builtin_amdgcn_readfirstlane(pr.j);
                if (p.same && pr.j <= pr.i) {
                    if (p.final_stage && pr.j == pr.i && tid == 0)
                        p.out[(long long)pr.i * p.ldo + pr.i] = p.kdiag[pr.i];
                    continue;
                }
            } else {
                if (tid < NP) {
                    unsigned iq = 0, jq = 0;
                    unit_pair(p, u + tid, iq, jq);
                    pair_tab[tid] = iq < p.n1 ? iq : p.n1 - 1;
                    pair_tab[kMaxNP + tid] = jq < p.n2 ? jq : p.n2 - 1;
                }
                pr.i = pr.j = 0;
                lds_barrier();
            }
            if constexpr (PID < 0) {
                for (int k = 0; k < p.nops; ++k) {
                    const cgp_net_op op = load_op(ops_c(p.ops) + k);
                    net_op<T, EX, DU, NP>(lds, op, p, pr, tid);
                    lds_barrier();
                }
            } else {
                prog_ops<T, DU, NP, PID, 0>(lds, p, pr, tid, prog_recs);
            }
            if (p.final_stage) {
                if constexpr (NP == 1) {
                    if (tid == 0) {
                        const T v = lds[p.final_slot];
                        p.out[(long long)pr.i * p.ldo + pr.j] = v;
                        if (p.same) p.out[(long long)pr.j * p.ldo + pr.i] = v;
                    }
                } else if (tid < NP) {
                    unsigned iq, jq;
                    if (u + tid < end && unit_pair(p, u + tid, iq, jq)) {
                        if (!p.same || jq > iq) {
                            const T v = lds[tid * p.lds_elems + p.final_slot];
                            p.out[(long long)iq * p.ldo + jq] = v;
                            if (p.same) p.out[(long long)jq * p.ldo + iq] = v;
                        } else if (jq == iq) {
                            p.out[(long long)iq * p.ldo + iq] = p.kdiag[iq];
                        }
                    }
                }
            }
        }
        lds_barrier();
    }
}

constexpr int net_wpe(long long lds_bytes, int cap = 5, int waves = kNT / 64) {
    const long long wg = (160LL * 1024) / (lds_bytes + kStaticLds);
    const long long w = wg * waves / 4;
    return w < 3 ? 3 : (w > cap ? cap : (int)w);
}
constexpr int kProgWpeMax = 5;

template <typename T, int NP>
const void* net_fn_np(bool du, long long lds_bytes) {
    switch (net_wpe(lds_bytes, 5, kNTof<NP> / 64)) {
    case 3: return du ? (const void*)net_kernel<T, false, true, 3, NP>
                      : (const void*)net_kernel<T, false, false, 3, NP>;
    case 4: return du ? (const void*)net_kernel<T, false, true, 4, NP>
                      : (const void*)net_kernel<T, false, false, 4, NP>;
    default:
        return du ? (const void*)net_kernel<T, false, true, 4, NP>
                  : (const void*)net_kernel<T, false, false, 5, NP>;
    }
}
template <typename T>
const void* net_fn(bool ex, bool du, int np, long long lds_bytes) {
    if (ex) {
        if (np != 1) return nullptr;
        return du ? (const void*)net_kernel<T, true, true, 3, 1>
                  : (const void*)net_kernel<T, true, false, 3, 1>;
    }
    if constexpr (sizeof(T) == 8) {
        switch (np) {
        case 1: return net_fn_np<T, 1>(du, lds_bytes);
        case 2: return net_fn_np<T, 2>(du, lds_bytes);
        case 4: return net_fn_np<T, 4>(du, lds_bytes);
        case 16: return net_fn_np<T, 16>(du, lds_bytes);
        default: return nullptr;
        }
    }
    switch (np) {
    case 1: return du ? (const void*)net_kernel<T, false, true, 4, 1>
                      : (const void*)net_kernel<T, false, false, 5, 1>;
    case 2: return du ? (const void*)net_kernel<T, false, true, 4, 2>
                      : (const void*)net_kernel<T, false, false, 5, 2>;
    case 4: return du ? (const void*)net_kernel<T, false, true, 4, 4>
                      : (const void*)net_kernel<T, false, false, 5, 4>;
    case 16: return du ? (const void*)net_kernel<T, false, true, 4, 16>
                       : (const void*)net_kernel<T, false, false, 5, 16>;
    default: return nullptr;
    }
}

template <typename T, int PID>
const void* prog_fn_one() {
    constexpr ProgInfo I = kProgs[PID];
    if constexpr ((I.sizes & (int)sizeof(T)) == 0) {
        return nullptr;
    } else {
        constexpr long long bytes =
            (long long)I.lds_elems * (long long)sizeof(T) * kUnitsOf<I.pairs>;
        constexpr int wpe = sizeof(T) == 8 ? net_wpe(bytes, kProgWpeMax, kNTof<I.pairs> / 64)
                                           : (I.dual ? 4 : 5);
        return (const void*)net_kernel<T, false, I.dual != 0, wpe, I.pairs, PID>;
    }
}
template <typename T>
const void* prog_fn(int pid) {
    switch (pid) {
#define CGP_PROG_CASE(k) \
    case k: return prog_fn_one<T, k>();
        CGP_NET_PROGRAMS(CGP_PROG_CASE)
#undef CGP_PROG_CASE
    default: return nullptr;
    }
}

int net_threads(int np) { return np == 2 ? kNTof<2> : kNT; }
int net_units(int np) { return np == 2 ? kUnitsOf<2> : np; }

int net_occupancy(const void* fn, int lds_bytes, int threads) {
    if (lds_bytes > 64 * 1024 &&
        hipFuncSetAttribute(fn, hipFuncAttributeMaxDynamicSharedMemorySize, lds_bytes) !=
            hipSuccess) {
        (void)hipGetLastError();
        return 0;
    }
    int n = 0;
    if (hipOccupancyMaxActiveBlocksPerMultiprocessor(&n, fn, threads, lds_bytes) != hipSuccess) {
        (void)hipGetLastError();
        return 0;
    }
    return n;
}

template <typename T>
int net_occupancy_for(int lds_bytes, int flags, int np) {
    const void* fn = net_fn<T>(flags & CGP_FLAG_EXACT_RELU, flags & CGP_FLAG_NET_DUAL, np,
                               (long long)lds_bytes * net_units(np));
    return fn ? net_occupancy(fn, lds_bytes * net_units(np), net_threads(np)) : 0;
}

unsigned long long* work_counters(hipStream_t s) {
    constexpr int kSlots = 64;
    struct Ring {
        unsigned long long* buf = nullptr;
        unsigned next = 0;
    };
    static std::mutex mu;
    static std::map<std::pair<int, hipStream_t>, Ring> rings;
    int dev = 0;
    if (stream_device(s, &dev) != hipSuccess) {
        (void)hipGetLastError();
        return nullptr;
    }
    unsigned long long* slot = nullptr;
    {
        std::lock_guard<std::mutex> lock(mu);
        Ring& r = rings[{dev, s}];
        if (!r.buf) {
            int cur = 0;
            hipError_t e = hipGetDevice(&cur);
            if (e == hipSuccess && cur != dev) e = hipSetDevice(dev);
            if (e == hipSuccess)
                e = hipMalloc(&r.buf, sizeof(unsigned long long) * 8 * kSlots);
            if (cur != dev) (void)hipSetDevice(cur);
            if (e != hipSuccess) {
                (void)hipGetLastError();
                r.buf = nullptr;
                return nullptr;
            }
        }
        slot = r.buf + 8 * (r.next++ % kSlots);
    }
    if (hipMemsetAsync(slot, 0, sizeof(unsigned long long) * 8, s) != hipSuccess) {
        (void)hipGetLastError();
        return nullptr;
    }
    return slot;
}

template <typename T>
int net_launch(const NetP<T>& p, bool ex, bool du, int np, long long lds_bytes, int program,
               void* stream) {
    const long long wg_bytes = lds_bytes * net_units(np);
    const void* fn = program > 0 && !ex ? prog_fn<T>(program - 1) : net_fn<T>(ex, du, np, wg_bytes);
    if (!fn) return fail(CGP_EINVAL, "net: no instantiation for %d pairs per workgroup", np);
    const int per_cu = net_occupancy(fn, (int)wg_bytes, net_threads(np));
    if (per_cu <= 0)
        return fail(CGP_EINVAL, "net: kernel cannot be resident with %lld B LDS", wg_bytes);
    const long long groups = (p.uend - p.ubeg + net_units(np) - 1) / net_units(np);
    long long grid = (long long)per_cu * device_cus();
    if (grid > groups) grid = groups;
    grid = (grid + 7) / 8 * 8;
    NetP<T> arg = p;
    hipStream_t s = as_stream(stream);
    arg.work = work_counters(s);
    if (!arg.work) return fail(CGP_EHIP, "net: work counters");
    void* args[] = {&arg};
    const hipError_t e = hipLaunchKernel(fn, dim3((unsigned)grid), dim3(net_threads(np)), args,
                                         (size_t)wg_bytes, s);
    if (e != hipSuccess) return fail(CGP_EHIP, "net_kernel launch: %s", hipGetErrorString(e));
    return check_launch("net_kernel");
}

template <typename T>
int net_impl(const cgp_net_args* a, void* stream) {
    if (!a) return fail(CGP_EINVAL, "net: args is NULL");
    if (!a->x || !a->y || !a->out || !a->ops || a->nops <= 0)
        return fail(CGP_EINVAL, "net: NULL pointer or empty op list");
    if (a->n1 <= 0 || a->n2 <= 0 || a->n1 >= (1LL << 31) || a->n2 >= (1LL << 31) ||
        a->ldo < a->n2)
        return fail(CGP_EINVAL, "net: bad sizes n1=%lld n2=%lld ldo=%lld", (long long)a->n1,
                    (long long)a->n2, (long long)a->ldo);
    if (a->same && (a->n1 != a->n2 || !a->kdiag))
        return fail(CGP_EINVAL, "net: same tile needs n1 == n2 and kdiag");
    if (a->channels <= 0 || a->h <= 0 || a->w <= 0)
        return fail(CGP_EINVAL, "net: bad image shape");
    const long long lds_bytes = (long long)a->lds_elems * (long long)sizeof(T);
    if (a->lds_elems <= 0 || lds_bytes + kStaticLds > 160 * 1024)
        return fail(CGP_EINVAL, "net: LDS footprint %lld bytes out of range", lds_bytes);
    if (a->final_slot < 0 || a->final_slot >= a->lds_elems || a->hs < 0 ||
        a->hs >= a->lds_elems || a->part < 0 || a->part + 2 > a->lds_elems)
        return fail(CGP_EINVAL, "net: slot offsets out of range");
    NetP<T> p;
    p.x = static_cast<const T*>(a->x);
    p.y = static_cast<const T*>(a->y);
    p.out = static_cast<T*>(a->out);
    p.kdiag = static_cast<const T*>(a->kdiag);
    p.ops = a->ops;
    p.ldo = a->ldo;
    p.n1 = (unsigned)a->n1;
    p.n2 = (unsigned)a->n2;
    p.nbi = (unsigned)((a->n1 + kST - 1) / kST);
    p.nbj = (unsigned)((a->n2 + kST - 1) / kST);
    const long long tiles = a->same ? (long long)p.nbi * (p.nbi + 1) / 2
                                    : (long long)p.nbi * p.nbj;
    if (tiles * kST * kST >= (1LL << 40)) return fail(CGP_EINVAL, "net: tile too large");
    p.units = tiles * kST * kST;
    p.nops = a->nops;
    p.channels = a->channels;
    p.hw_in = a->h * a->w;
    p.same = a->same;
    p.final_slot = a->final_slot;
    p.hs = a->hs;
    p.part = a->part;
    p.lds_elems = a->lds_elems;
    p.exact = (a->flags & CGP_FLAG_EXACT_RELU) ? 1 : 0;
    const int np = a->pairs <= 0 ? 1 : a->pairs;
    if (np != 1 && np != 2 && np != 4 && np != kMaxNP)
        return fail(CGP_EINVAL, "net: %d pairs per workgroup (1, 2, 4 or 16)", np);
    if (lds_bytes * net_units(np) + kStaticLds > 160 * 1024)
        return fail(CGP_EINVAL, "net: %d pairs need %lld B LDS (+ %lld B static)", np,
                    lds_bytes * net_units(np), kStaticLds);
    if (np > 1 && (a->n1 > a->n2 ? a->n1 : a->n2) * (8LL * net_threads(np) / np) *
                          (long long)sizeof(T) >= (1LL << 32))
        return fail(CGP_EINVAL, "net: %lld images too many for %d pairs per workgroup",
                    (long long)(a->n1 > a->n2 ? a->n1 : a->n2), np);
    if (a->unit_begin == 0 && a->unit_end == 0) {
        p.ubeg = 0;
        p.uend = p.units;
    } else {
        p.ubeg = a->unit_begin;
        p.uend = a->unit_end;
    }
    if (p.ubeg < 0 || p.uend > p.units || p.ubeg >= p.uend || p.ubeg % np)
        return fail(CGP_EINVAL, "net: unit range [%lld, %lld) of %lld", (long long)p.ubeg,
                    (long long)p.uend, (long long)p.units);
    p.final_stage = a->final_stage;
    const bool du = (a->flags & CGP_FLAG_NET_DUAL) != 0;
    const int prog = a->program;
    if (prog < 0 || prog > kNumProgs)
        return fail(CGP_EINVAL, "net: program %d of %d", prog, kNumProgs);
    if (prog > 0) {
        const ProgInfo& I = kProgs[prog - 1];
        if (I.nops != a->nops || I.pairs != np || I.dual != (du ? 1 : 0) ||
            I.lds_elems != a->lds_elems || !(I.sizes & (int)sizeof(T)))
            return fail(CGP_EINVAL, "net: program %d does not fit this op list", prog);
    }
    return net_launch<T>(p, p.exact != 0, du, np, lds_bytes, prog, stream);
}

}

extern "C" {

int cgp_net_geometry(int32_t h, int32_t w, int32_t ho, int32_t wo, int32_t taps,
                     int32_t stride, int32_t offset) {
    for (int k = 0; k < kNumGeo; ++k) {
        const GeoRow& g = kGeoTable[k];
        if (g.h == h && g.w == w && g.ho == ho && g.wo == wo && g.taps == taps &&
            g.s == stride && g.off == offset)
            return k;
    }
    return -1;
}

int cgp_net_resolution(int32_t h, int32_t w) { return res_index(h, w); }

size_t cgp_net_op_size(void) { return sizeof(cgp_net_op); }
size_t cgp_net_args_size(void) { return sizeof(cgp_net_args); }

int cgp_net_supertile(void) { return kST; }
int cgp_net_var_form(void) { return kNetVarForm; }

int cgp_net_units(int32_t pairs) { return net_units(pairs <= 0 ? 1 : pairs); }

int cgp_net_hs_elems(int32_t code) {
    return (code >= 0 && code < kNumGeo) ? kGeoTable[code].hs_elems : -1;
}

int cgp_net_occupancy(int32_t lds_bytes, int32_t f64, int32_t flags, int32_t pairs) {
    if (pairs <= 0) pairs = 1;
    if (lds_bytes <= 0 || (long long)lds_bytes * pairs > 160 * 1024) return 0;
    return f64 ? net_occupancy_for<double>(lds_bytes, flags, pairs)
               : net_occupancy_for<float>(lds_bytes, flags, pairs);
}

int cgp_net_static_lds(void) { return (int)kStaticLds; }

int cgp_net_validate(const cgp_net_op* ops, int32_t nops, int32_t pairs) {
    if (!ops || nops <= 0) return fail(CGP_EINVAL, "net_validate: NULL or empty op list");
    const int np = pairs <= 0 ? 1 : pairs;
    auto geo = [](const cgp_net_op& r) -> const GeoRow* {
        const int g = r.code & CGP_NET_CODE_GEOMETRY;
        return r.kind == CGP_NET_CONV && r.code >= 0 && g < kNumGeo ? &kGeoTable[g] : nullptr;
    };
    for (int k = 0; k < nops; ++k) {
        const cgp_net_op& r = ops[k];
        const bool sum = r.kind == CGP_NET_CONV && r.code >= 0 && (r.code & CGP_NET_CODE_SUM);
        const bool from = r.kind == CGP_NET_CONV && r.code >= 0 && (r.code & CGP_NET_CODE_FROM_SUM);
        if (sum) {
            const GeoRow* g = geo(r);
            const bool point = g && g->taps == 1 && g->off == 0;
            const bool reduce = g && g->ho == 1 && g->wo == 1 && g->off == 0 &&
                                g->taps == g->h && g->taps == g->w;
            if (!g || g->taps <= 3 || point || reduce)
                return fail(CGP_EINVAL, "net_validate: op %d: CGP_NET_CODE_SUM needs a separable "
                                        "conv (more than 3 taps, not pointwise, not a reduction)", k);
            if (r.add >= 0 || r.dst2 >= 0)
                return fail(CGP_EINVAL, "net_validate: op %d: CGP_NET_CODE_SUM with an addend or "
                                        "a second output", k);
            if (np > 2)
                return fail(CGP_EINVAL, "net_validate: op %d: CGP_NET_CODE_SUM in a %d-pair stage "
                                        "(one pair per workgroup or half only)", k, np);
            if (k + 1 >= nops || !(ops[k + 1].kind == CGP_NET_CONV && ops[k + 1].code >= 0 &&
                                   (ops[k + 1].code & CGP_NET_CODE_FROM_SUM)) ||
                ops[k + 1].src != r.dst)
                return fail(CGP_EINVAL, "net_validate: op %d: CGP_NET_CODE_SUM not followed by the "
                                        "CGP_NET_CODE_FROM_SUM reduction of its map", k);
            for (int m = k + 2; m < nops; ++m)
                if (ops[m].src == r.dst || ops[m].add == r.dst)
                    return fail(CGP_EINVAL, "net_validate: op %d reads the map of SUM op %d, "
                                            "which is never stored", m, k);
        }
        if (from) {
            const GeoRow* g = geo(r);
            const bool reduce = g && g->ho == 1 && g->wo == 1 && g->off == 0 &&
                                g->taps == g->h && g->taps == g->w;
            if (!reduce || np > 2)
                return fail(CGP_EINVAL, "net_validate: op %d: CGP_NET_CODE_FROM_SUM needs a "
                                        "one-pair full-map reduction", k);
            if (k == 0 || !(ops[k - 1].kind == CGP_NET_CONV && ops[k - 1].code >= 0 &&
                            (ops[k - 1].code & CGP_NET_CODE_SUM)))
                return fail(CGP_EINVAL, "net_validate: op %d: CGP_NET_CODE_FROM_SUM without a "
                                        "CGP_NET_CODE_SUM conv before it", k);
        }
    }
    return CGP_OK;
}

int cgp_net_program(const cgp_net_op* ops, int32_t nops, int32_t pairs, int32_t flags,
                    int32_t lds_elems, int32_t itemsize) {
    if (!ops || nops <= 0) return 0;
    return prog_match(ops, nops, pairs <= 0 ? 1 : pairs, (flags & CGP_FLAG_NET_DUAL) ? 1 : 0,
                      lds_elems, itemsize);
}

int cgp_net_f64(const cgp_net_args* args, void* stream) { return net_impl<double>(args, stream); }
int cgp_net_f32(const cgp_net_args* args, void* stream) { return net_impl<float>(args, stream); }

}
```

include/cnngp.h:

```cpp
#ifndef CNNGP_H
#define CNNGP_H

#include <stddef.h>
#include <stdint.h>

#ifdef __cplusplus
extern "C" {
#endif

#define CGP_ABI_VERSION 12

#define CGP_OK 0
#define CGP_EINVAL 1001
#define CGP_EHIP 1002
#define CGP_EBLAS 1003

#define CGP_PRE_NONE 0
#define CGP_PRE_RELU 1
#define CGP_PRE_MOMENTS 2
#define CGP_POST_NONE 0
#define CGP_POST_RELU 1

#define CGP_FLAG_EXACT_RELU 1
#define CGP_FLAG_GENERIC_CONV 2

int cgp_abi_version(void);
double cgp_net_xvar_scale(void);
#define CGP_VAR_FORM_SCALED 0
#define CGP_VAR_FORM_RSQRT 1
int cgp_net_var_form(void);
const char* cgp_last_error(void);
size_t cgp_conv_args_size(void);
size_t cgp_relu_args_size(void);
int cgp_device_count(void);
int cgp_selftest(void);

int cgp_moments_xy_f64(const double* x, const double* y, int64_t n1, int64_t n2,
                       int32_t c, int32_t hw, int32_t diag, double* xy, void* stream);
int cgp_moments_xy_f32(const float* x, const float* y, int64_t n1, int64_t n2,
                       int32_t c, int32_t hw, int32_t diag, float* xy, void* stream);
int cgp_moments_var_f64(const double* x, const double* y, int64_t n1, int64_t n2,
                        int32_t c, int32_t hw, double* xx, double* yy, void* stream);
int cgp_moments_var_f32(const float* x, const float* y, int64_t n1, int64_t n2,
                        int32_t c, int32_t hw, float* xx, float* yy, void* stream);

typedef struct cgp_conv_args {
    const void* in;
    const void* in_y;
    void* out;
    const void* addend;
    const void* pre_xx;
    const void* pre_yy;
    const void* post_xx;
    const void* post_yy;
    int64_t nmaps;
    int64_t n1, n2;
    int32_t h, w, ho, wo;
    int32_t taps, offset, stride, dilation;
    int32_t channels;
    int32_t pre, post;
    int32_t same, diag;
    int32_t maps_per_block;
    int32_t flags;
    int32_t reserved;
    double weight, bias;
} cgp_conv_args;
int cgp_conv_f64(const cgp_conv_args* args, void* stream);
int cgp_conv_f32(const cgp_conv_args* args, void* stream);

typedef struct cgp_relu_args {
    const void* xy;
    void* out;
    const void* addend;
    const void* xx;
    const void* yy;
    int64_t nmaps, n1, n2;
    int32_t hw, same, diag, flags;
} cgp_relu_args;
int cgp_relu_f64(const cgp_relu_args* args, void* stream);
int cgp_relu_f32(const cgp_relu_args* args, void* stream);

typedef struct cgp_relu_ntk_args {
    const void* xy;
    const void* theta;
    void* out_xy;
    void* out_theta;
    const void* xx;
    const void* yy;
    int64_t nmaps, n1, n2;
    int32_t hw, same, diag, flags;
} cgp_relu_ntk_args;
size_t cgp_relu_ntk_args_size(void);
int cgp_relu_ntk_f64(const cgp_relu_ntk_args* args, void* stream);
int cgp_relu_ntk_f32(const cgp_relu_ntk_args* args, void* stream);

int cgp_var_relu_f64(const double* xx, const double* yy, int64_t n1, int64_t n2, int32_t hw,
                     int32_t same, double* xx_out, double* yy_out, void* stream);
int cgp_var_relu_f32(const float* xx, const float* yy, int64_t n1, int64_t n2, int32_t hw,
                     int32_t same, float* xx_out, float* yy_out, void* stream);

typedef struct cgp_erf_args {
    const void* xy;
    const void* theta;
    void* out_xy;
    void* out_theta;
    const void* addend;
    const void* xx;
    const void* yy;
    int64_t nmaps, n1, n2;
    int32_t hw, same, diag, flags;
} cgp_erf_args;
size_t cgp_erf_args_size(void);
int cgp_erf_f64(const cgp_erf_args* args, void* stream);
int cgp_erf_f32(const cgp_erf_args* args, void* stream);

int cgp_var_erf_f64(const double* xx, const double* yy, int64_t n1, int64_t n2, int32_t hw,
                    int32_t same, double* xx_out, double* yy_out, void* stream);
int cgp_var_erf_f32(const float* xx, const float* yy, int64_t n1, int64_t n2, int32_t hw,
                    int32_t same, float* xx_out, float* yy_out, void* stream);

int cgp_axpby_f64(double alpha, const double* a, double beta, const double* b, double* out,
                  int64_t n, void* stream);
int cgp_axpby_f32(double alpha, const float* a, double beta, const float* b, float* out,
                  int64_t n, void* stream);

int cgp_scale_batch_f64(int32_t count, const double* const* src, double* const* dst,
                        const int64_t* n, double alpha, void* stream);
int cgp_rsqrt_batch_f64(int32_t count, const double* const* src, double* const* dst,
                        const int64_t* n, void* stream);

int cgp_cast_f32_f64(const float* in, double* out, int64_t n, void* stream);
int cgp_transpose_f64(const double* src, int64_t rows, int64_t cols, double* dst, void* stream);

int cgp_chol_solve_f64(double* k, int64_t n, int64_t ldk, double* bt, int64_t nrhs,
                       int64_t ldb, double jitter, int64_t* info, void* stream);
int cgp_chol_last_phases(void* stream, double* ms);
int cgp_chol_solve_f64_timed(double* k, int64_t n, int64_t ldk, double* bt, int64_t nrhs,
                             int64_t ldb, double jitter, int64_t* info, double* phase_ms,
                             void* stream);
int cgp_sym_mirror_f64(double* k, int64_t n, int64_t ldk, double* diag, void* stream);
int cgp_sym_residual_f64(const double* k, int64_t n, int64_t ldk, const double* diag,
                         const double* x, double* r, int64_t nrhs, int64_t ldx, double* sumsq,
                         void* stream);
int cgp_gemm_f64(const double* a, const double* b, double* c, int64_t m, int64_t n,
                 int64_t kdim, void* stream);
int cgp_pred_var_f64(const double* k, int64_t n, int64_t ldk, double* kxz, int64_t m,
                     int64_t ldz, const double* kz_diag, double* var, void* stream);
int cgp_argmax_rows_f64(const double* a, int64_t rows, int64_t cols, int64_t* out,
                        void* stream);


#define CGP_NET_CONV 0
#define CGP_NET_RELU 1
#define CGP_NET_MOMENTS 2
#define CGP_NET_LINEAR 3
#define CGP_NET_LOAD 4
#define CGP_NET_STORE 5
#define CGP_NET_CODE_HS_CLEAN 0x100
#define CGP_NET_CODE_SUM 0x200
#define CGP_NET_CODE_FROM_SUM 0x400
#define CGP_NET_CODE_GEOMETRY 0xff

typedef struct cgp_net_op {
    int32_t kind;
    int32_t code;
    int32_t src, dst, add;
    int32_t ws_in, ws_out;
    int32_t relu;
    int32_t h, w;
    uint32_t div_m, div_s;
    int32_t dst2;
    int32_t zero_halo;
    double weight, bias;
    const void* var_x;
    const void* var_y;
    const void* var2_x;
    const void* var2_y;
} cgp_net_op;

typedef struct cgp_net_args {
    const void* x;
    const void* y;
    void* out;
    const void* kdiag;
    const cgp_net_op* ops;
    int64_t n1, n2, ldo;
    int32_t nops, channels, h, w;
    int32_t same;
    int32_t final_slot;
    int32_t hs;
    int32_t lds_elems;
    int32_t flags;
    int32_t pairs;
    int64_t unit_begin;
    int64_t unit_end;
    int32_t final_stage;
    int32_t program;
    int32_t part;
} cgp_net_args;

#define CGP_VAR_MOMENTS 0
#define CGP_VAR_CONV 1
#define CGP_VAR_HALF 2
#define CGP_VAR_SUM 3
typedef struct cgp_var_op {
    int32_t kind;
    int32_t dst;
    int32_t src[4];
    int32_t h, w, ho, wo;
    int32_t taps, offset, stride, dilation;
    int64_t store;
    int64_t qstore;
    double weight, bias;
    double coef[4];
} cgp_var_op;
typedef struct cgp_var_args {
    const void* x;
    const void* y;
    void* out;
    const cgp_var_op* ops;
    int64_t n1, n2;
    int64_t store_total;
    int32_t nops, channels, h, w;
    int32_t lds_elems;
    int32_t scratch;
} cgp_var_args;
size_t cgp_var_op_size(void);
size_t cgp_var_args_size(void);
int cgp_var_chain_f64(const cgp_var_args* args, void* stream);
int cgp_var_chain_f32(const cgp_var_args* args, void* stream);

int cgp_net_geometry(int32_t h, int32_t w, int32_t ho, int32_t wo, int32_t taps,
                     int32_t stride, int32_t offset);
int cgp_net_hs_elems(int32_t code);
int cgp_net_supertile(void);
size_t cgp_net_op_size(void);
size_t cgp_net_args_size(void);
int cgp_net_resolution(int32_t h, int32_t w);
#define CGP_FLAG_NET_DUAL 4
int cgp_net_occupancy(int32_t lds_bytes, int32_t f64, int32_t flags, int32_t pairs);
int cgp_net_units(int32_t pairs);
int cgp_net_program(const cgp_net_op* ops, int32_t nops, int32_t pairs, int32_t flags,
                    int32_t lds_elems, int32_t itemsize);
int cgp_net_validate(const cgp_net_op* ops, int32_t nops, int32_t pairs);
int cgp_net_static_lds(void);
int cgp_net_f64(const cgp_net_args* args, void* stream);
int cgp_net_f32(const cgp_net_args* args, void* stream);

#ifdef __cplusplus
}
#endif

#endif
```

Before: 118.1 million pairs/s.

## Add lean fp64 ReLU path with compile-time program analysis dropping caps and abs

Adds a compile-time analysis of fused network programs. It decides which ReLU outputs can be stored halved, so the c+|c| term becomes c with pre-halved polynomial coefficients and doubled downstream weights, and which ReLUs can skip the Y overflow cap. At runtime, a per-block check on weight and bias ranges selects a lean walk variant, instantiated from a shared include. This removes a few ALU ops per ReLU element in the fp64 kernel, at the cost of a second kernel body, larger code, and reliance on the range assumptions holding.

Measured after the change: 120.4 million pairs/s (median of 6 runs). 2.0% higher.

```diff
diff --git a/cnn-gp_amd/cnn_gp/_native.py b/cnn-gp_amd/cnn_gp/_native.py
--- a/cnn-gp_amd/cnn_gp/_native.py
+++ b/cnn-gp_amd/cnn_gp/_native.py
@@ -169,6 +169,8 @@
     "cgp_net_args_size": (ctypes.c_size_t, []),
     "cgp_net_occupancy": (_i32, [_i32, _i32, _i32, _i32]),
     "cgp_net_program": (_i32, [_vp, _i32, _i32, _i32, _i32, _i32]),
+    "cgp_net_program_lean": (_i32, [_vp, _i32, _i32, _i32, _i32, _i32,
+                                    ctypes.POINTER(_i32), ctypes.POINTER(_i32)]),
     "cgp_net_validate": (_i32, [_vp, _i32, _i32]),
     "cgp_net_static_lds": (_i32, []),
     "cgp_net_f64": (_i32, [ctypes.POINTER(NetArgs), _vp]),
diff --git a/cnn-gp_amd/csrc/cgp_common.h b/cnn-gp_amd/csrc/cgp_common.h
--- a/cnn-gp_amd/csrc/cgp_common.h
+++ b/cnn-gp_amd/csrc/cgp_common.h
@@ -147,6 +147,16 @@
 }
 static __constant__ PolyCoef kReluPolyTabD = poly_coef(false);
 static __constant__ PolyCoef kReluPolyTabDq = poly_coef(true);
+#ifndef CGP_RELU_LEAN
+#define CGP_RELU_LEAN 1
+#endif
+constexpr bool kReluLean = CGP_RELU_LEAN != 0 && CGP_RELU_ONE_ROOT != 0;
+template <class C>
+constexpr C half_coef(C t) {
+    for (double& v : t.c) v *= 0.5;
+    return t;
+}
+static __constant__ PolyCoef kReluPolyTabDqH = half_coef(poly_coef(true));
 
 template <int D>
 struct AdaptCoef {
@@ -165,19 +175,23 @@
 static __constant__ AdaptCoef<kReluAdaptDeg0> kReluAdaptTab0 = adapt_coef<kReluAdaptDeg0>(kReluAdaptP0);
 static __constant__ AdaptCoef<kReluAdaptDeg1> kReluAdaptTab1 = adapt_coef<kReluAdaptDeg1>(kReluAdaptP1);
 static __constant__ AdaptCoef<kReluAdaptDeg2> kReluAdaptTab2 = adapt_coef<kReluAdaptDeg2>(kReluAdaptP2);
+static __constant__ AdaptCoef<kReluAdaptDeg0> kReluAdaptTab0H = half_coef(adapt_coef<kReluAdaptDeg0>(kReluAdaptP0));
+static __constant__ AdaptCoef<kReluAdaptDeg1> kReluAdaptTab1H = half_coef(adapt_coef<kReluAdaptDeg1>(kReluAdaptP1));
+static __constant__ AdaptCoef<kReluAdaptDeg2> kReluAdaptTab2H = half_coef(adapt_coef<kReluAdaptDeg2>(kReluAdaptP2));
 
 typedef const __attribute__((address_space(4))) double* ConstD;
 struct PolyTab {
     ConstD d, dq;
     ConstD a0, a1, a2;
 };
+template <bool HALF = false>
 __device__ __forceinline__ PolyTab poly_table() {
     ConstD p = (ConstD)kReluPolyTabD.c;
-    ConstD q = (ConstD)kReluPolyTabDq.c;
+    ConstD q = (ConstD)(HALF ? kReluPolyTabDqH.c : kReluPolyTabDq.c);
     asm volatile("" : "+s"(p), "+s"(q));
-    ConstD a0 = (ConstD)kReluAdaptTab0.c;
-    ConstD a1 = (ConstD)kReluAdaptTab1.c;
-    ConstD a2 = (ConstD)kReluAdaptTab2.c;
+    ConstD a0 = (ConstD)(HALF ? kReluAdaptTab0H.c : kReluAdaptTab0.c);
+    ConstD a1 = (ConstD)(HALF ? kReluAdaptTab1H.c : kReluAdaptTab1.c);
+    ConstD a2 = (ConstD)(HALF ? kReluAdaptTab2H.c : kReluAdaptTab2.c);
     asm volatile("" : "+s"(a0), "+s"(a1), "+s"(a2));
     return PolyTab{p, q, a0, a1, a2};
 }
@@ -260,17 +274,21 @@
     for (int r = 1; r < R; ++r) m = m > vote_hi(u[r]) ? m : vote_hi(u[r]);
     return m;
 }
-template <int R, bool QIN, int AD = 0>
+template <int R, bool QIN, int AD = 0, bool NOCAP = false, bool HALF = false>
 __device__ __forceinline__ void relu_q_n(double (&c)[R], const double (&v1q)[R],
                                          const double (&v2)[R], const PolyTab& tab,
                                          unsigned long long seg = ~0ull) {
+    static_assert(CGP_RELU_ONE_ROOT || (!NOCAP && !HALF), "lean forms: one-root form only");
     double sx[R], u[R], p[R];
 #if CGP_RELU_ONE_ROOT
     double Y[R];
 #pragma unroll
     for (int r = 0; r < R; ++r) {
         if constexpr (!QIN) c[r] *= 0.25;
-        Y[r] = __builtin_fmin(v1q[r] * v2[r], kYMax);
+        if constexpr (NOCAP)
+            Y[r] = v1q[r] * v2[r];
+        else
+            Y[r] = __builtin_fmin(v1q[r] * v2[r], kYMax);
     }
 #pragma unroll
     for (int r = 0; r < R; ++r) {
@@ -352,7 +370,12 @@
         horner_q<R, kReluPolyDegD>(p, u, tab.dq);
     }
 #pragma unroll
-    for (int r = 0; r < R; ++r) c[r] = __builtin_fma(sx[r], p[r], c[r] + __builtin_fabs(c[r]));
+    for (int r = 0; r < R; ++r) {
+        if constexpr (HALF)
+            c[r] = __builtin_fma(sx[r], p[r], c[r]);
+        else
+            c[r] = __builtin_fma(sx[r], p[r], c[r] + __builtin_fabs(c[r]));
+    }
 }
 typedef float cgp_f2 __attribute__((ext_vector_type(2)));
 __device__ __forceinline__ cgp_f2 relu_fast2(cgp_f2 c, cgp_f2 v1, cgp_f2 v2) {
diff --git a/cnn-gp_amd/csrc/net_walk.inc b/cnn-gp_amd/csrc/net_walk.inc
--- /dev/null
+++ b/cnn-gp_amd/csrc/net_walk.inc
@@ -0,0 +1,106 @@
+    for (long long u = advance(); u < end; u = advance()) {
+        if (tid == 0) grab = atomicAdd(ctr, 1ull);
+        Pairs pr;
+        pr.tab = pair_tab;
+        pr.u0 = u;
+        pr.red = red_part;
+        if constexpr (NP == 2) {
+            const int q = __builtin_amdgcn_readfirstlane(tid >> 7);
+            unsigned iq = 0, jq = 0;
+            bool vq = false, wq = false, any = false;
+#pragma unroll
+            for (int s = 0; s < UN; ++s) {
+                unsigned is = 0, js = 0;
+                const bool vs = u + s < end && unit_pair(p, u + s, is, js);
+                const bool ws = vs && !(p.same && js <= is);
+                any |= ws;
+                if (s == q) {
+                    iq = is;
+                    jq = js;
+                    vq = vs;
+                    wq = ws;
+                }
+            }
+            if (!any) {
+                if (p.final_stage && p.same && (tid & (kNT - 1)) == 0 && vq && jq == iq)
+                    p.out[(long long)iq * p.ldo + iq] = p.kdiag[iq];
+                continue;
+            }
+            Pairs ph;
+            ph.tab = pair_tab;
+            ph.u0 = u + q;
+            ph.red = red_part + q * (kNT / 64);
+            ph.i = __builtin_amdgcn_readfirstlane(vq ? iq : 0u);
+            ph.j = __builtin_amdgcn_readfirstlane(vq ? jq : 0u);
+            T* lh = lds + q * p.lds_elems;
+            const int ht = tid & (kNT - 1);
+            if constexpr (PID < 0) {
+                for (int k = 0; k < p.nops; ++k) {
+                    const cgp_net_op op = load_op(ops_c(p.ops) + k);
+                    net_op<T, EX, DU, 1>(lh, op, p, ph, ht);
+                    lds_barrier();
+                }
+            } else {
+                prog_ops<T, DU, 1, PID, 0, CGP_WALK_LEAN>(lh, p, ph, ht, prog_recs);
+            }
+            if (p.final_stage && ht == 0 && vq) {
+                if (wq) {
+                    const T v = lh[p.final_slot];
+                    p.out[(long long)ph.i * p.ldo + ph.j] = v;
+                    if (p.same) p.out[(long long)ph.j * p.ldo + ph.i] = v;
+                } else if (ph.j == ph.i) {
+                    p.out[(long long)ph.i * p.ldo + ph.i] = p.kdiag[ph.i];
+                }
+            }
+        } else {
+            if constexpr (NP == 1) {
+                if (!unit_pair(p, u, pr.i, pr.j)) continue;
+                pr.i = __builtin_amdgcn_readfirstlane(pr.i);
+                pr.j = __builtin_amdgcn_readfirstlane(pr.j);
+                if (p.same && pr.j <= pr.i) {
+                    if (p.final_stage && pr.j == pr.i && tid == 0)
+                        p.out[(long long)pr.i * p.ldo + pr.i] = p.kdiag[pr.i];
+                    continue;
+                }
+            } else {
+                if (tid < NP) {
+                    unsigned iq = 0, jq = 0;
+                    unit_pair(p, u + tid, iq, jq);
+                    pair_tab[tid] = iq < p.n1 ? iq : p.n1 - 1;
+                    pair_tab[kMaxNP + tid] = jq < p.n2 ? jq : p.n2 - 1;
+                }
+                pr.i = pr.j = 0;
+                lds_barrier();
+            }
+            if constexpr (PID < 0) {
+                for (int k = 0; k < p.nops; ++k) {
+                    const cgp_net_op op = load_op(ops_c(p.ops) + k);
+                    net_op<T, EX, DU, NP>(lds, op, p, pr, tid);
+                    lds_barrier();
+                }
+            } else {
+                prog_ops<T, DU, NP, PID, 0, CGP_WALK_LEAN>(lds, p, pr, tid, prog_recs);
+            }
+            if (p.final_stage) {
+                if constexpr (NP == 1) {
+                    if (tid == 0) {
+                        const T v = lds[p.final_slot];
+                        p.out[(long long)pr.i * p.ldo + pr.j] = v;
+                        if (p.same) p.out[(long long)pr.j * p.ldo + pr.i] = v;
+                    }
+                } else if (tid < NP) {
+                    unsigned iq, jq;
+                    if (u + tid < end && unit_pair(p, u + tid, iq, jq)) {
+                        if (!p.same || jq > iq) {
+                            const T v = lds[tid * p.lds_elems + p.final_slot];
+                            p.out[(long long)iq * p.ldo + jq] = v;
+                            if (p.same) p.out[(long long)jq * p.ldo + iq] = v;
+                        } else if (jq == iq) {
+                            p.out[(long long)iq * p.ldo + iq] = p.kdiag[iq];
+                        }
+                    }
+                }
+            }
+        }
+        lds_barrier();
+    }
diff --git a/cnn-gp_amd/csrc/netfuse.hip b/cnn-gp_amd/csrc/netfuse.hip
--- a/cnn-gp_amd/csrc/netfuse.hip
+++ b/cnn-gp_amd/csrc/netfuse.hip
@@ -233,14 +233,15 @@
 template <typename T, bool EX>
 constexpr bool kQuarter = !EX && sizeof(T) == 8;
 
-template <bool EXACT, bool QIN, typename T, int R, int AD = 0>
+template <bool EXACT, bool QIN, typename T, int R, int AD = 0, bool NC = false, bool HF = false>
 __device__ __forceinline__ void relu_n(T (&v)[R], const T (&u1)[R], const T (&u2)[R],
                                        const PolyTab& tab, unsigned long long seg = ~0ull) {
+    static_assert(!(NC || HF) || (!EXACT && sizeof(T) == 8), "lean ReLU forms: fp64 closed form");
     if constexpr (EXACT) {
 #pragma unroll
         for (int k = 0; k < R; ++k) v[k] = relu_exact_inl(v[k], u1[k], u2[k]);
     } else if constexpr (sizeof(T) == 8) {
-        relu_q_n<R, QIN, AD>(v, u1, u2, tab, seg);
+        relu_q_n<R, QIN, AD, NC, HF>(v, u1, u2, tab, seg);
     } else {
         relu_fast_n<R>(v, u1, u2, tab);
     }
@@ -261,12 +262,12 @@
     return -1;
 }
 
-template <typename T, bool EX, bool DU, int R, int AD = 0>
+template <typename T, bool EX, bool DU, int R, int AD = 0, bool NC = false, bool HF = false>
 __device__ __forceinline__ void net_out(T* __restrict__ lds, const cgp_net_op& op, T (&v)[R],
                                         const int (&at)[R], const bool (&ok)[R],
                                         const T (&u1)[R], const T (&u2)[R],
                                         const PolyTab& tab, unsigned long long seg = ~0ull) {
-    if (op.relu) relu_n<EX, kQuarter<T, EX>, T, R, AD>(v, u1, u2, tab, seg);
+    if (op.relu) relu_n<EX, kQuarter<T, EX>, T, R, AD, NC, HF>(v, u1, u2, tab, seg);
     if (op.add >= 0) {
 #pragma unroll
         for (int k = 0; k < R; ++k)
@@ -372,12 +373,13 @@
 #ifndef CGP_NET_RES_UNDEF
 #define CGP_NET_RES_UNDEF 1
 #endif
-template <typename T, bool EX, bool DU, class G, bool PRE = false>
+template <typename T, bool EX, bool DU, class G, bool PRE = false, bool NC = false,
+          bool HF = false>
 __device__ __forceinline__ void net_conv(T* __restrict__ lds, const cgp_net_op& op,
                                          const NetP<T>& p, const Pairs& pr) {
     constexpr int NP = G::NP;
     const int tid = opaque_tid();
-    const PolyTab tab = poly_table();
+    const PolyTab tab = poly_table<HF>();
     const T qs = !PRE && kQuarter<T, EX> && op.relu ? T(0.25) : T(1);
     const T w = T(op.weight) * qs, b = T(op.bias) * qs;
     const int arena = NP == 1 ? 0 : p.lds_elems;
@@ -426,7 +428,7 @@
                 u1[0] = vs0.ldx(0);
                 u2[0] = vs0.ldy(0);
             }
-            net_out<T, EX, DU, 1>(lds, op, v, at, ok, u1, u2, tab);
+            net_out<T, EX, DU, 1, 0, NC, HF>(lds, op, v, at, ok, u1, u2, tab);
         }
     } else if constexpr (G::REDUCE) {
         prio_alu<NP, G::HW>();
@@ -455,7 +457,7 @@
                 u1[0] = vs.ldx(0);
                 u2[0] = vs.ldy(0);
             }
-            net_out<T, EX, DU, 1>(lds, op, v, at, ok, u1, u2, tab);
+            net_out<T, EX, DU, 1, 0, NC, HF>(lds, op, v, at, ok, u1, u2, tab);
         }
     } else if constexpr (G::POINT) {
         prio_alu<NP, G::HW>();
@@ -477,7 +479,7 @@
             u2[k] = (vs.on && ok[k]) ? vs.ldy((unsigned)pc) : T(1);
             v[k] = fma_t(w, src[q * arena + (r * G::S) * wsi + c * G::S], b);
         }
-        net_out<T, EX, DU, KP, NP == 1 ? 1 : 0>(lds, op, v, at, ok, u1, u2, tab);
+        net_out<T, EX, DU, KP, NP == 1 ? 1 : 0, NC, HF>(lds, op, v, at, ok, u1, u2, tab);
     } else if constexpr (G::DIRECT) {
         constexpr int NVT = NP * G::NV;
         T u1[G::KV][G::R3], u2[G::KV][G::R3];
@@ -551,9 +553,9 @@
                     at[k] = q * arena + (g3 * G::R3 + k) * wso + c;
                     ok[k] = true;
                 }
-                net_out<T, EX, DU, G::R3, kAdaptOf<NP>>(lds, op, res[kv], at, ok, u1[kv],
-                                                        u2[kv], tab,
-                                                        NP == 1 ? ~0ull : vote_lanes<G::NV, NP>(it));
+                net_out<T, EX, DU, G::R3, kAdaptOf<NP>, NC, HF>(
+                    lds, op, res[kv], at, ok, u1[kv], u2[kv], tab,
+                    NP == 1 ? ~0ull : vote_lanes<G::NV, NP>(it));
             }
         }
     } else {
@@ -638,14 +640,14 @@
                     ok[k] = true;
                 }
                 if (to_sum) {
-                    if (op.relu) relu_n<EX, kQuarter<T, EX>, T, G::R3, 1>(v, u1[kv], u2[kv], tab);
+                    if (op.relu)
+                        relu_n<EX, kQuarter<T, EX>, T, G::R3, 1, NC, HF>(v, u1[kv], u2[kv], tab);
 #pragma unroll
                     for (int k = 0; k < G::R3; ++k) sacc += v[k];
                 } else {
-                    net_out<T, EX, DU, G::R3, kAdaptOf<NP>>(lds, op, v, at, ok, u1[kv], u2[kv],
-                                                            tab,
-                                                            NP == 1 ? ~0ull
-                                                                    : vote_lanes<G::NV, NP>(it));
+                    net_out<T, EX, DU, G::R3, kAdaptOf<NP>, NC, HF>(
+                        lds, op, v, at, ok, u1[kv], u2[kv], tab,
+                        NP == 1 ? ~0ull : vote_lanes<G::NV, NP>(it));
                 }
             }
         }
@@ -999,12 +1001,172 @@
     static constexpr GeoRow g = kGeoTable[o.code & CGP_NET_CODE_GEOMETRY];
     using G = NG<g.h, g.w, g.ho, g.wo, g.taps, g.s, g.off, NP>;
 };
-template <typename T, bool DU, int NP, int PID, int K>
+__host__ __device__ inline bool lean_rec_ok(double w, double b) {
+    return w >= 0.0 && w <= 0x1p60 && b >= 0x1p-60 && b <= 0x1p60;
+}
+constexpr int kMaxProgOps = 24;
+struct LeanOp {
+    bool nocap = false, half = false, dbl = false;
+};
+struct ProgLean {
+    LeanOp op[kMaxProgOps] = {};
+    unsigned dbl_mask = 0;
+    int capfree = 0, addfree = 0;
+    int nend = 0, end_lo[4] = {}, end_hi[4] = {};
+    bool bad = false;
+};
+struct LeanFact {
+    int lo = 0, hi = 0;
+    bool nonneg = false, halved = false;
+};
+constexpr bool lean_overlap(int lo, int hi, int lo2, int hi2) { return lo < hi2 && lo2 < hi; }
+constexpr bool op_is_sum(const ProgOp& o) {
+    return o.kind == CGP_NET_CONV && (o.code & CGP_NET_CODE_SUM) != 0;
+}
+constexpr int op_src_hi(const ProgOp& o) {
+    if (o.kind == CGP_NET_CONV) return o.src + kGeoTable[o.code & CGP_NET_CODE_GEOMETRY].h * o.ws_in;
+    if (o.kind == CGP_NET_RELU || o.kind == CGP_NET_LINEAR || o.kind == CGP_NET_STORE)
+        return o.src + o.h * o.ws_in;
+    return o.src;
+}
+constexpr bool op_reads_add(const ProgOp& o) {
+    return (o.kind == CGP_NET_CONV || o.kind == CGP_NET_RELU) ? o.add >= 0
+                                                              : o.kind == CGP_NET_LINEAR;
+}
+constexpr bool op_writes_dst(const ProgOp& o) { return o.kind != CGP_NET_STORE; }
+constexpr int op_ext(const ProgOp& o) { return o.h * o.ws_out; }
+constexpr bool lean_can_halve(const ProgOp* ops, int n, int k, int lo, int hi, bool* end) {
+    *end = false;
+    for (int m = k + 1; m < n; ++m) {
+        const ProgOp& r = ops[m];
+        if (op_reads_add(r) && lean_overlap(lo, hi, r.add, r.add + op_ext(r))) return false;
+        if (lean_overlap(lo, hi, r.src, op_src_hi(r)) &&
+            !(r.kind == CGP_NET_CONV && r.src == lo && op_src_hi(r) <= hi))
+            return false;
+        if (op_is_sum(r)) continue;
+        if (op_writes_dst(r) && lean_overlap(lo, hi, r.dst, r.dst + op_ext(r))) {
+            if (r.dst <= lo && r.dst + op_ext(r) >= hi) return true;
+            return false;
+        }
+        if (r.dst2 >= 0 && lean_overlap(lo, hi, r.dst2, r.dst2 + op_ext(r))) {
+            if (r.dst2 <= lo && r.dst2 + op_ext(r) >= hi) return true;
+            return false;
+        }
+    }
+    if (op_is_sum(ops[k]))
+        return k + 1 < n && ops[k + 1].kind == CGP_NET_CONV &&
+               (ops[k + 1].code & CGP_NET_CODE_FROM_SUM) != 0 && ops[k + 1].src == lo;
+    *end = true;
+    return true;
+}
+constexpr ProgLean prog_lean(int pid) {
+    ProgLean L{};
+    const ProgInfo I = kProgs[pid];
+    const ProgOp* ops = kProgOps + I.first;
+    if (I.nops > kMaxProgOps) {
+        L.bad = true;
+        return L;
+    }
+    if (I.pairs > 2 || I.dual) return L;
+    constexpr int kMaxFacts = 8;
+    LeanFact f[kMaxFacts] = {};
+    int nf = 0;
+    auto find = [&](int lo, int hi) -> const LeanFact* {
+        for (int n = 0; n < nf; ++n)
+            if (f[n].lo == lo && hi <= f[n].hi) return &f[n];
+        return nullptr;
+    };
+    auto touches_halved = [&](int lo, int hi) {
+        for (int n = 0; n < nf; ++n)
+            if (f[n].halved && lean_overlap(lo, hi, f[n].lo, f[n].hi)) return true;
+        return false;
+    };
+    auto write = [&](int lo, int hi, bool nonneg, bool halved) {
+        int m = 0;
+        for (int n = 0; n < nf; ++n)
+            if (!lean_overlap(lo, hi, f[n].lo, f[n].hi)) f[m++] = f[n];
+        nf = m;
+        if (!nonneg) return;
+        if (nf == kMaxFacts) {
+            if (halved) L.bad = true;
+            return;
+        }
+        f[nf].lo = lo;
+        f[nf].hi = hi;
+        f[nf].nonneg = nonneg;
+        f[nf].halved = halved;
+        ++nf;
+    };
+    for (int k = 0; k < I.nops; ++k) {
+        const ProgOp& o = ops[k];
+        const int ext = op_ext(o);
+        const LeanFact* fs = find(o.src, op_src_hi(o));
+        const LeanFact* fa = op_reads_add(o) ? find(o.add, o.add + ext) : nullptr;
+        const bool add_nn = !op_reads_add(o) || (fa && fa->nonneg);
+        if (op_reads_add(o) && touches_halved(o.add, o.add + ext)) L.bad = true;
+        if (o.kind != CGP_NET_CONV && op_src_hi(o) > o.src && touches_halved(o.src, op_src_hi(o)))
+            L.bad = true;
+        if (o.kind == CGP_NET_CONV) {
+            if (touches_halved(o.src, op_src_hi(o)) && !(fs && fs->halved)) L.bad = true;
+            const bool src_nn = fs && fs->nonneg;
+            L.op[k].dbl = fs && fs->halved;
+            if (L.op[k].dbl) L.dbl_mask |= 1u << k;
+            bool half = false;
+            if (o.relu) {
+                L.op[k].nocap = true;
+                ++L.capfree;
+                bool end = false;
+                half = src_nn && o.add < 0 && o.dst2 < 0 &&
+                       lean_can_halve(ops, I.nops, k, o.dst, o.dst + ext, &end);
+                if (half && end) {
+                    if (L.nend == 4) {
+                        half = false;
+                    } else {
+                        L.end_lo[L.nend] = o.dst;
+                        L.end_hi[L.nend++] = o.dst + ext;
+                    }
+                }
+                L.op[k].half = half;
+                L.addfree += half;
+            }
+            write(o.dst, o.dst + ext, (o.relu || src_nn) && add_nn, half);
+            if (o.dst2 >= 0) write(o.dst2, o.dst2 + ext, true, false);
+        } else if (o.kind == CGP_NET_RELU) {
+            write(o.dst, o.dst + ext, add_nn, false);
+        } else if (o.kind == CGP_NET_LINEAR) {
+            write(o.dst, o.dst + ext, false, false);
+            if (o.dst2 >= 0) write(o.dst2, o.dst2 + ext, true, false);
+        } else if (o.kind == CGP_NET_MOMENTS || o.kind == CGP_NET_LOAD) {
+            write(o.dst, o.dst + ext, false, false);
+        }
+    }
+    return L;
+}
+template <int PID>
+struct LeanOf {
+    static constexpr ProgLean L = prog_lean(PID < 0 ? 0 : PID);
+    static_assert(!L.bad, "prog_lean: a program the slot walk does not cover");
+};
+#define CGP_LEAN_ROW(k) LeanOf<k>::L,
+constexpr ProgLean kLeanTab[] = {CGP_NET_PROGRAMS(CGP_LEAN_ROW)};
+#undef CGP_LEAN_ROW
+bool lean_final_clash(int pid, int final_slot) {
+    const ProgLean& L = kLeanTab[pid];
+    for (int n = 0; n < L.nend; ++n)
+        if (final_slot >= L.end_lo[n] && final_slot < L.end_hi[n]) return true;
+    return false;
+}
+template <typename T, int PID>
+constexpr bool kLeanProg = PID >= 0 && kReluLean && sizeof(T) == 8 &&
+                           LeanOf<PID>::L.capfree + LeanOf<PID>::L.addfree > 0;
+
+template <typename T, bool DU, int NP, int PID, int K, bool LEAN = false>
 __device__ __forceinline__ void prog_ops(T* __restrict__ lds, const NetP<T>& p, const Pairs& pr,
                                          int tid, const ProgRec* recs) {
     constexpr ProgInfo I = kProgs[PID];
     if constexpr (K < I.nops) {
         constexpr ProgOp o = kProgOps[I.first + K];
+        constexpr LeanOp lean = LEAN ? LeanOf<PID>::L.op[K] : LeanOp{};
         const cgp_net_op op = prog_op<PID, K>(recs);
         if constexpr (o.zero_halo != 0) {
 #pragma unroll
@@ -1018,8 +1180,9 @@
             }
         }
         if constexpr (o.kind == CGP_NET_CONV) {
-            net_conv<T, false, DU, typename ProgGeo<PID, K, NP>::G, kNetPrescale>(lds, op, p,
-                                                                                 pr);
+            static_assert(!lean.half || (o.relu && o.add < 0 && o.dst2 < 0), "halved output");
+            net_conv<T, false, DU, typename ProgGeo<PID, K, NP>::G, kNetPrescale, lean.nocap,
+                     lean.half>(lds, op, p, pr);
         } else if constexpr (o.kind == CGP_NET_RELU || o.kind == CGP_NET_LINEAR ||
                              o.kind == CGP_NET_MOMENTS) {
             net_elem<T, false, DU, o.kind, o.h, o.w, NP>(lds, op, p, pr);
@@ -1031,10 +1194,9 @@
                 net_move<T, o.kind, NP>(lds, op, p, pr);
         }
         lds_barrier();
-        prog_ops<T, DU, NP, PID, K + 1>(lds, p, pr, tid, recs);
-    }
-}
-
+        prog_ops<T, DU, NP, PID, K + 1, LEAN>(lds, p, pr, tid, recs);
+    }
+}
 int prog_match(const cgp_net_op* ops, int nops, int pairs, int dual, int lds_elems,
                int itemsize) {
     for (int k = 0; k < kNumProgs; ++k) {
@@ -1068,16 +1230,27 @@
     if (tid < UN * (kNT / 64)) red_part[tid] = T(0);
     __shared__ ProgRec prog_recs[kRecsOf<PID>];
     __shared__ long long next_u[2];
-    static_assert(sizeof(pair_tab) + sizeof(red_part) + sizeof(prog_recs) + sizeof(next_u) <=
-                      kStaticLds,
+    __shared__ int lean_flag;
+    static_assert(sizeof(pair_tab) + sizeof(red_part) + sizeof(prog_recs) + sizeof(next_u) +
+                      sizeof(lean_flag) <= kStaticLds,
                   "static LDS beyond the reserve the host checks count (kStaticLds)");
     if constexpr (PID >= 0) {
+        const ProgOp* po = kProgOps + kProgs[PID < 0 ? 0 : PID].first;
         for (int k = tid; k < kRecsOf<PID>; k += kNTof<NP>) {
             const cgp_net_op& r = p.ops[k];
-            const ProgOp& o = kProgOps[kProgs[PID < 0 ? 0 : PID].first + k];
+            const ProgOp& o = po[k];
             const double qs =
                 kNetPrescale && kQuarter<T, false> && o.kind == CGP_NET_CONV && o.relu ? 0.25 : 1.0;
-            prog_recs[k] = ProgRec{r.weight * qs, r.bias * qs, r.var_x, r.var_y, r.var2_x,
+            double ws = qs;
+            if constexpr (kLeanProg<T, PID>) {
+                bool ok = true;
+                for (int n = 0; n < kRecsOf<PID>; ++n)
+                    if (po[n].kind == CGP_NET_CONV)
+                        ok = ok && lean_rec_ok(p.ops[n].weight, p.ops[n].bias);
+                if (ok && ((LeanOf<PID>::L.dbl_mask >> k) & 1u)) ws *= 2.0;
+                if (k == 0) lean_flag = ok;
+            }
+            prog_recs[k] = ProgRec{r.weight * ws, r.bias * qs, r.var_x, r.var_y, r.var2_x,
                                    r.var2_y};
         }
     }
@@ -1098,112 +1271,17 @@
         adv ^= 1;
         return v;
     };
-    for (long long u = advance(); u < end; u = advance()) {
-        if (tid == 0) grab = atomicAdd(ctr, 1ull);
-        Pairs pr;
-        pr.tab = pair_tab;
-        pr.u0 = u;
-        pr.red = red_part;
-        if constexpr (NP == 2) {
-            const int q = __builtin_amdgcn_readfirstlane(tid >> 7);
-            unsigned iq = 0, jq = 0;
-            bool vq = false, wq = false, any = false;
-#pragma unroll
-            for (int s = 0; s < UN; ++s) {
-                unsigned is = 0, js = 0;
-                const bool vs = u + s < end && unit_pair(p, u + s, is, js);
-                const bool ws = vs && !(p.same && js <= is);
-                any |= ws;
-                if (s == q) {
-                    iq = is;
-                    jq = js;
-                    vq = vs;
-                    wq = ws;
-                }
-            }
-            if (!any) {
-                if (p.final_stage && p.same && (tid & (kNT - 1)) == 0 && vq && jq == iq)
-                    p.out[(long long)iq * p.ldo + iq] = p.kdiag[iq];
-                continue;
-            }
-            Pairs ph;
-            ph.tab = pair_tab;
-            ph.u0 = u + q;
-            ph.red = red_part + q * (kNT / 64);
-            ph.i = __builtin_amdgcn_readfirstlane(vq ? iq : 0u);
-            ph.j = __builtin_amdgcn_readfirstlane(vq ? jq : 0u);
-            T* lh = lds + q * p.lds_elems;
-            const int ht = tid & (kNT - 1);
-            if constexpr (PID < 0) {
-                for (int k = 0; k < p.nops; ++k) {
-                    const cgp_net_op op = load_op(ops_c(p.ops) + k);
-                    net_op<T, EX, DU, 1>(lh, op, p, ph, ht);
-                    lds_barrier();
-                }
-            } else {
-                prog_ops<T, DU, 1, PID, 0>(lh, p, ph, ht, prog_recs);
-            }
-            if (p.final_stage && ht == 0 && vq) {
-                if (wq) {
-                    const T v = lh[p.final_slot];
-                    p.out[(long long)ph.i * p.ldo + ph.j] = v;
-                    if (p.same) p.out[(long long)ph.j * p.ldo + ph.i] = v;
-                } else if (ph.j == ph.i) {
-                    p.out[(long long)ph.i * p.ldo + ph.i] = p.kdiag[ph.i];
-                }
-            }
-        } else {
-            if constexpr (NP == 1) {
-                if (!unit_pair(p, u, pr.i, pr.j)) continue;
-                pr.i = __builtin_amdgcn_readfirstlane(pr.i);
-                pr.j = __builtin_amdgcn_readfirstlane(pr.j);
-                if (p.same && pr.j <= pr.i) {
-                    if (p.final_stage && pr.j == pr.i && tid == 0)
-                        p.out[(long long)pr.i * p.ldo + pr.i] = p.kdiag[pr.i];
-                    continue;
-                }
-            } else {
-                if (tid < NP) {
-                    unsigned iq = 0, jq = 0;
-                    unit_pair(p, u + tid, iq, jq);
-                    pair_tab[tid] = iq < p.n1 ? iq : p.n1 - 1;
-                    pair_tab[kMaxNP + tid] = jq < p.n2 ? jq : p.n2 - 1;
-                }
-                pr.i = pr.j = 0;
-                lds_barrier();
-            }
-            if constexpr (PID < 0) {
-                for (int k = 0; k < p.nops; ++k) {
-                    const cgp_net_op op = load_op(ops_c(p.ops) + k);
-                    net_op<T, EX, DU, NP>(lds, op, p, pr, tid);
-                    lds_barrier();
-                }
-            } else {
-                prog_ops<T, DU, NP, PID, 0>(lds, p, pr, tid, prog_recs);
-            }
-            if (p.final_stage) {
-                if constexpr (NP == 1) {
-                    if (tid == 0) {
-                        const T v = lds[p.final_slot];
-                        p.out[(long long)pr.i * p.ldo + pr.j] = v;
-                        if (p.same) p.out[(long long)pr.j * p.ldo + pr.i] = v;
-                    }
-                } else if (tid < NP) {
-                    unsigned iq, jq;
-                    if (u + tid < end && unit_pair(p, u + tid, iq, jq)) {
-                        if (!p.same || jq > iq) {
-                            const T v = lds[tid * p.lds_elems + p.final_slot];
-                            p.out[(long long)iq * p.ldo + jq] = v;
-                            if (p.same) p.out[(long long)jq * p.ldo + iq] = v;
-                        } else if (jq == iq) {
-                            p.out[(long long)iq * p.ldo + iq] = p.kdiag[iq];
-                        }
-                    }
-                }
-            }
-        }
-        lds_barrier();
-    }
+    if constexpr (kLeanProg<T, PID>) {
+        if (__builtin_amdgcn_readfirstlane(lean_flag) != 0) {
+#define CGP_WALK_LEAN true
+#include "net_walk.inc"
+#undef CGP_WALK_LEAN
+            return;
+        }
+    }
+#define CGP_WALK_LEAN false
+#include "net_walk.inc"
+#undef CGP_WALK_LEAN
 }
 
 constexpr int net_wpe(long long lds_bytes, int cap = 5, int waves = kNT / 64) {
@@ -1439,6 +1517,10 @@
         if (I.nops != a->nops || I.pairs != np || I.dual != (du ? 1 : 0) ||
             I.lds_elems != a->lds_elems || !(I.sizes & (int)sizeof(T)))
             return fail(CGP_EINVAL, "net: program %d does not fit this op list", prog);
+        if (kReluLean && sizeof(T) == 8 && !p.exact && a->final_stage &&
+            lean_final_clash(prog - 1, a->final_slot))
+            return fail(CGP_EINVAL, "net: final slot %d of program %d is a map slot",
+                        (int)a->final_slot, prog);
     }
     return net_launch<T>(p, p.exact != 0, du, np, lds_bytes, prog, stream);
 }
@@ -1539,6 +1621,22 @@
                       lds_elems, itemsize);
 }
 
+int cgp_net_program_lean(const cgp_net_op* ops, int32_t nops, int32_t pairs, int32_t flags,
+                         int32_t lds_elems, int32_t itemsize, int32_t* capfree,
+                         int32_t* addfree) {
+    if (!kReluLean || !ops || nops <= 0 || itemsize != 8 || (flags & CGP_FLAG_EXACT_RELU))
+        return 0;
+    const int k = prog_match(ops, nops, pairs <= 0 ? 1 : pairs,
+                             (flags & CGP_FLAG_NET_DUAL) ? 1 : 0, lds_elems, itemsize);
+    if (k <= 0) return 0;
+    for (int n = 0; n < nops; ++n)
+        if (ops[n].kind == CGP_NET_CONV && !lean_rec_ok(ops[n].weight, ops[n].bias)) return 0;
+    const ProgLean& L = kLeanTab[k - 1];
+    if (capfree) *capfree = L.capfree;
+    if (addfree) *addfree = L.addfree;
+    return 1;
+}
+
 int cgp_net_f64(const cgp_net_args* args, void* stream) { return net_impl<double>(args, stream); }
 int cgp_net_f32(const cgp_net_args* args, void* stream) { return net_impl<float>(args, stream); }
 
diff --git a/include/cnngp.h b/include/cnngp.h
--- a/include/cnngp.h
+++ b/include/cnngp.h
@@ -242,6 +242,9 @@
 int cgp_net_units(int32_t pairs);
 int cgp_net_program(const cgp_net_op* ops, int32_t nops, int32_t pairs, int32_t flags,
                     int32_t lds_elems, int32_t itemsize);
+int cgp_net_program_lean(const cgp_net_op* ops, int32_t nops, int32_t pairs, int32_t flags,
+                         int32_t lds_elems, int32_t itemsize, int32_t* capfree,
+                         int32_t* addfree);
 int cgp_net_validate(const cgp_net_op* ops, int32_t nops, int32_t pairs);
 int cgp_net_static_lds(void);
 int cgp_net_f64(const cgp_net_args* args, void* stream);
```
